# anisanazim/Movie-Recommendation-Engine

Measured on AMD Instinct MI355X. Metric: item embeddings/sec + top-K ANN queries/sec, ML-25M d=256, 1/2/4/8 GPU, higher is better.
Workload: dtype f64 cdf / f32 features / fp4 sign planes (exact integer Hamming); 1 GPU; SYN-25M (ML-25M-shaped: U=162541 M=59047 R=25000095), F=128 H=256 d=256, 2 GCN layers, W=100 L=2 T=10, LSH 512-bit, 10000 queries K=11, rng=numpy (the reference's np.random MT19937 stream generated on device: neighbour ids bit-exact with the reference CPU path); global_items=59047, queries=10000, parallelism=item-shard x1

## Files before the change

### include/pinsage_hip.h

```cpp
#ifndef PINSAGE_HIP_H
#define PINSAGE_HIP_H

#include <stddef.h>
#include <stdint.h>

#ifdef __cplusplus
extern "C" {
#endif

#define PS_OK 0
#define PS_EINVAL (-1)
#define PS_ELAUNCH (-2)
#define PS_EWORKSPACE (-3)
#define PS_EUNSUPPORTED (-4)

#define PS_RNG_STREAM 0
#define PS_RNG_PHILOX 1
#define PS_RNG_STREAM_RAW 2

#define PS_RNG_STREAM_WALKS 3

#define PS_WALK_HALF_BUCKETS 0x100

typedef void *ps_stream_t;

int ps_abi_version(void);
const char *ps_error_string(int code);

size_t ps_csr_build_workspace_bytes(int64_t E, int64_t V);
int ps_csr_build(const int64_t *src, const int64_t *dst, const float *w, int64_t E, int64_t V,
                 int64_t *rowptr, int32_t *col, double *wsorted,
                 void *workspace, size_t workspace_bytes, ps_stream_t stream);

int ps_cdf_build(const int64_t *rowptr, const double *wsorted, int64_t V, double *cdf, ps_stream_t stream);

int ps_guide_build(const int64_t *rowptr, const double *cdf, int64_t V, uint32_t *nodeinfo, int32_t *guide,
                   ps_stream_t stream);

int ps_pack_edges(const int32_t *col, const double *cdf, const int32_t *guide, int64_t E, void *packed,
                  ps_stream_t stream);

int ps_bucket_build(const int64_t *rowptr, const int32_t *col, const double *cdf, const int32_t *guide, int64_t V,
                    int64_t E, void *buckets, ps_stream_t stream);

int ps_bucket_build_half(const int64_t *rowptr, const int32_t *col, const double *cdf, const int32_t *guide, int64_t V,
                         int64_t E, void *buckets, ps_stream_t stream);

int ps_dest_info_build(const int32_t *col, const uint32_t *nodeinfo, int64_t E, int64_t V, void *dest_info, ps_stream_t stream);

int ps_graph_stats(const int64_t *rowptr, const int32_t *col, int64_t E, int64_t V, int64_t *flags,
                   ps_stream_t stream);

int ps_walk_sample(const int64_t *rowptr, const int32_t *col, const double *cdf, int64_t V,
                   const int64_t *starts, int64_t B, int W, int L, int T,
                   int rng_mode, const double *uniforms, const int64_t *uoff,
                   uint64_t seed, uint32_t call, const uint32_t *nodeinfo, const int32_t *guide,
                   const void *packed, const void *buckets, const void *dest_info,
                   int32_t *ids, int32_t *counts, int32_t *nvalid, ps_stream_t stream);

int ps_walk_sample_layers(const int64_t *rowptr, const int32_t *col, const double *cdf, int64_t V,
                          const int64_t *starts, int64_t B, int W, int L, int T,
                          int rng_mode, const double *uniforms, const int64_t *uoff, int64_t layer_stride,
                          uint64_t seed, uint32_t call, const uint32_t *nodeinfo, const int32_t *guide,
                          const void *packed, const void *buckets, const void *dest_info, int layers,
                          int32_t *ids, int32_t *counts, int32_t *nvalid, ps_stream_t stream);

int ps_walk_paths(const int64_t *rowptr, const int32_t *col, const double *cdf, int64_t V,
                  const int64_t *starts, int64_t B, int L, int rng_mode, const double *uniforms,
                  const int64_t *uoff, uint64_t seed, uint32_t call, int walk_mod,
                  const uint32_t *nodeinfo, const int32_t *guide, int32_t *paths, ps_stream_t stream);

int ps_uniform_offsets(const int64_t *rowptr, int64_t V, const int64_t *starts, int64_t B, int W, int L,
                       int64_t *uoff, int64_t *total, ps_stream_t stream);

int ps_mt19937_chunk_log2(void);
int ps_mt19937_window_shift(void);
int ps_mt19937_raw_stream(const uint32_t *state_in, int pos_in, int64_t n, uint32_t *raw, uint32_t *state_out,
                          int32_t *pos_out, const uint32_t *jump_polys, int jump_levels, const uint32_t *radix_polys,
                          int radix_levels, const uint32_t *window_polys, int n_window, const int64_t *ranges,
                          int n_ranges, void *workspace, size_t workspace_bytes, ps_stream_t stream);
size_t ps_mt19937_workspace_bytes(int64_t skip, int64_t n);
int ps_mt19937_random_sample(const uint32_t *state_in, int pos_in, int64_t skip, int64_t n, double *out,
                             uint32_t *state_out, int32_t *pos_out, const uint32_t *jump_polys, int jump_levels,
                             const uint32_t *radix_polys, int radix_levels, const uint32_t *window_polys, int n_window,
                             void *workspace, size_t workspace_bytes, ps_stream_t stream);

int ps_importance_pool(const float *x, int64_t N, int H, const int32_t *ids, const int32_t *counts,
                       const float *wts, const int32_t *nvalid, int64_t B, int T, int64_t max_idx,
                       int renorm, float *out, ps_stream_t stream);

#define PS_RELU 1
#define PS_L2NORM 2
#define PS_WPERM 4
int ps_permute_k(const float *W, int64_t rows, int K, int ld, float *out, ps_stream_t stream);
int ps_linear(const float *x, int64_t M, int K, const float *W, int ldw, const float *b, int N,
              const float *x2, int K2, const float *W2, int ldw2, int flags, float *y, ps_stream_t stream);

int ps_lsh_encode(const float *x, int64_t N, int D, const float *A, int nbits, uint8_t *codes, int flags, ps_stream_t stream);

size_t ps_hamming_topk_workspace_bytes(int64_t nq, int64_t N, int cs, int k);
int ps_hamming_topk(const uint8_t *qcodes, int64_t nq, const uint8_t *codes, int64_t N, int cs, int k,
                    int64_t id_offset, int32_t *dist, int64_t *ids,
                    void *workspace, size_t workspace_bytes, ps_stream_t stream);

size_t ps_lsh_planes_bytes(int64_t n, int cs);
int ps_lsh_expand(const uint8_t *codes, int64_t n, int cs, void *planes, ps_stream_t stream);
size_t ps_hamming_topk_mfma_workspace_bytes(int64_t nq, int64_t N, int cs, int k);
int ps_hamming_topk_mfma(const void *qplanes, int64_t nq, const void *dbplanes, int64_t N, int cs, int k,
                         int64_t id_offset, int32_t *dist, int64_t *ids,
                         void *workspace, size_t workspace_bytes, ps_stream_t stream);
int ps_hamming_topk_mfma_codes(const uint8_t *qcodes, int64_t nq, const void *dbplanes, int64_t N, int cs, int k,
                               int64_t id_offset, int32_t *dist, int64_t *ids,
                               void *workspace, size_t workspace_bytes, ps_stream_t stream);

int ps_topk_merge(const int32_t *dist_in, const int64_t *ids_in, int P, int64_t nq, int k,
                  int32_t *dist, int64_t *ids, ps_stream_t stream);
int ps_topk_merge_strided(const int32_t *dist_in, int64_t dist_stride, const int64_t *ids_in, int64_t ids_stride,
                          int P, int64_t nq, int k, int32_t *dist, int64_t *ids, ps_stream_t stream);

size_t ps_dot_topk_workspace_bytes(int64_t nq, int64_t N, int D, int k);
int ps_dot_topk(const float *E, int64_t N, int D, const int64_t *qidx, int64_t nq, int k, int exclude_self,
                float *vals, int64_t *ids, void *workspace, size_t workspace_bytes, ps_stream_t stream);

size_t ps_l2_topk_workspace_bytes(int64_t nq, int64_t N, int D, int k);
int ps_l2_topk(const float *X, int64_t N, int D, const float *Q, int64_t nq, int k, const int32_t *assign,
               const uint32_t *probe, int words, float *dist, int64_t *ids, void *workspace,
               size_t workspace_bytes, ps_stream_t stream);

size_t ps_ivf_topk_workspace_bytes(int64_t nq, int64_t N, int D, int k, int nlist, int nprobe, int64_t max_list);
int ps_ivf_topk(const float *X, int64_t N, int D, const int64_t *list_ptr, int nlist, int64_t max_list,
                const int64_t *item_ids, const float *Q, int64_t nq, const int32_t *probes, int nprobe, int k,
                float *dist, int64_t *ids, void *workspace, size_t workspace_bytes, ps_stream_t stream);

int ps_spmm_csr(const int64_t *rowptr, const int32_t *col, const float *val, const float *x, int64_t N, int H,
                int64_t V, int64_t E, float *out, ps_stream_t stream);

#ifdef __cplusplus
}
#endif
#endif
```

### movie-recommendation-engine_amd/csrc/dense_mfma.hip

```cpp
#include "ps_common.h"
#include <type_traits>

#ifndef PS_GEMM_DEBUG
#define PS_GEMM_DEBUG 0
#endif

#ifndef PS_GEMM_SPREAD
#define PS_GEMM_SPREAD 1
#endif

#if PS_GEMM_DEBUG & 64
__device__ unsigned long long ps_gemm_trace_buf[4096 * 4 * 48];
#define PS_TRACE(slot) do { if (lane == 0 && blockIdx.x < 4096 && (slot) < 48) \
    ps_gemm_trace_buf[((size_t)blockIdx.x * 4 + (wv & 3)) * 48 + (slot)] = __builtin_readcyclecounter(); } while (0)
extern "C" int ps_debug_gemm_trace(unsigned long long *host, int clear) {
    if (clear) { static unsigned long long z[4096 * 4 * 48]; return (int)hipMemcpyToSymbol(HIP_SYMBOL(ps_gemm_trace_buf), z, sizeof z); }
    return (int)hipMemcpyFromSymbol(host, HIP_SYMBOL(ps_gemm_trace_buf), sizeof(unsigned long long) * 4096 * 4 * 48);
}
#else
#define PS_TRACE(slot) do {} while (0)
#endif

namespace {

typedef float f32x16 __attribute__((ext_vector_type(16)));
typedef float f32x4 __attribute__((ext_vector_type(4)));


struct GemmArgs {
    const float *x;  int64_t M; int K;  const float *W;  int ldw;
    const float *x2; int K2;            const float *W2; int ldw2;
    const float *bias; int N; int flags;
    float *y;
    uint8_t *codes; int cs;
    const int64_t *grp;
};

__device__ __forceinline__ void load8(const float *base, bool row_ok, int k, int K, bool vec_ok, float (&v)[8]) {
    if (row_ok && vec_ok && k + 8 <= K) {
        const float4 a = *reinterpret_cast<const float4 *>(base + k);
        const float4 b = *reinterpret_cast<const float4 *>(base + k + 4);
        v[0] = a.x; v[1] = a.y; v[2] = a.z; v[3] = a.w; v[4] = b.x; v[5] = b.y; v[6] = b.z; v[7] = b.w;
    } else {
#pragma unroll
        for (int j = 0; j < 8; ++j) v[j] = (row_ok && k + j < K) ? base[k + j] : 0.f;
    }
}

#define PS_DPP_ACC(v, ctrl, rows) \
    (v) += __builtin_bit_cast(float, __builtin_amdgcn_update_dpp(0, __builtin_bit_cast(int, (v)), (ctrl), (rows), 0xf, true))
__device__ __forceinline__ float half_sum32(float v) {
    PS_DPP_ACC(v, 0xB1, 0xf);
    PS_DPP_ACC(v, 0x4E, 0xf);
    PS_DPP_ACC(v, 0x141, 0xf);
    PS_DPP_ACC(v, 0x140, 0xf);
    PS_DPP_ACC(v, 0x142, 0xa);
    return v;
}
#undef PS_DPP_ACC

#define PS_DPP_ADD(v, ctrl) \
    ((v) + __builtin_bit_cast(float, __builtin_amdgcn_update_dpp(0, __builtin_bit_cast(int, (v)), (ctrl), 0xf, 0xf, true)))
template <int NV>
__device__ __forceinline__ float transpose_sum32(float (&v)[NV], int lane) {
    static_assert(NV == 16 || NV == 32, "one or two 32-row tiles per wave");
    const bool p1 = ((lane ^ (lane >> 2)) & 1) != 0, p2 = (((lane >> 1) ^ (lane >> 2)) & 1) != 0;
    const bool p3 = (((lane >> 2) ^ (lane >> 3)) & 1) != 0, p4 = ((lane >> 3) & 1) != 0;
#pragma unroll
    for (int j = 0; j < NV / 2; ++j) {
        const float lo = PS_DPP_ADD(v[2 * j], 0xB1), hi = PS_DPP_ADD(v[2 * j + 1], 0xB1);
        v[j] = p1 ? hi : lo;
    }
#pragma unroll
    for (int j = 0; j < NV / 4; ++j) {
        const float lo = PS_DPP_ADD(v[2 * j], 0x4E), hi = PS_DPP_ADD(v[2 * j + 1], 0x4E);
        v[j] = p2 ? hi : lo;
    }
#pragma unroll
    for (int j = 0; j < NV / 8; ++j) {
        const float lo = PS_DPP_ADD(v[2 * j], 0x141), hi = PS_DPP_ADD(v[2 * j + 1], 0x141);
        v[j] = p3 ? hi : lo;
    }
#pragma unroll
    for (int j = 0; j < NV / 16; ++j) {
        const float lo = PS_DPP_ADD(v[2 * j], 0x140), hi = PS_DPP_ADD(v[2 * j + 1], 0x140);
        v[j] = p4 ? hi : lo;
    }
    const float x = v[0], y = NV == 32 ? v[1] : v[0];
    const auto sw = __builtin_amdgcn_permlane16_swap(__builtin_bit_cast(unsigned, x), __builtin_bit_cast(unsigned, y), false, false);
    const unsigned s0 = sw[0], s1 = sw[1];
    return __builtin_bit_cast(float, s0) + __builtin_bit_cast(float, s1);
}
#undef PS_DPP_ADD

template <bool PIN>
__device__ __forceinline__ void stash_item(float *d, f32x4 lo, f32x4 hi) {
    if (PIN) asm volatile("" : "+v"(lo), "+v"(hi));
    *reinterpret_cast<f32x4 *>(d) = f32x4{lo[0], lo[2], hi[0], hi[2]};
    *reinterpret_cast<f32x4 *>(d + 4) = f32x4{lo[1], lo[3], hi[1], hi[3]};
}
template <bool PIN>
__device__ __forceinline__ void stash_item_stored(float *d, f32x4 lo, f32x4 hi) {
    if (PIN) asm volatile("" : "+v"(lo), "+v"(hi));
    *reinterpret_cast<f32x4 *>(d) = lo;
    *reinterpret_cast<f32x4 *>(d + 4) = hi;
}

template <int WM, int WN, int TM, int TN, int EPI>
__device__ __forceinline__ void gemm_epilogue(const GemmArgs &g, f32x16 (&acc)[TM][TN], int64_t m0, int n0, float *sRed, float *sNrm) {
    constexpr int BM = WM * TM * 32, BN = WN * TN * 32, NT = WM * WN * 64;
    const int tid = threadIdx.x, lane = tid & 63, wv = tid >> 6;
    const int wm = wv / WN, wn = wv % WN, li = lane & 31, lh = lane >> 5;
    (void)BN; (void)wv;
    PS_TRACE(40);
    if (EPI == 1) {
        uint32_t *codes32 = reinterpret_cast<uint32_t *>(g.codes);
        const int words = g.cs >> 2;
#pragma unroll
        for (int a = 0; a < TM; ++a)
#pragma unroll
            for (int b = 0; b < TN; ++b) {
                const int colbase = n0 + (wn * TN + b) * 32;
                const bool col_ok = colbase + li < g.N;
#pragma unroll
                for (int r = 0; r < 16; ++r) {
                    const uint64_t mask = __ballot(col_ok && acc[a][b][r] >= 0.f);
                    const int64_t row = m0 + (wm * TM + a) * 32 + (r & 3) + 8 * (r >> 2) + 4 * lh;
                    if (li == 0 && row < g.M && colbase < g.N)
                        codes32[row * words + (colbase >> 5)] = lh ? (uint32_t)(mask >> 32) : (uint32_t)mask;
                }
            }
        PS_TRACE(41);
        return;
    }

    const bool relu = (g.flags & PS_RELU) && !(PS_GEMM_DEBUG & 8), l2 = (g.flags & PS_L2NORM) && !(PS_GEMM_DEBUG & 8);
    if (PS_GEMM_DEBUG & 32) {
        float s = 0.f;
#pragma unroll
        for (int a = 0; a < TM; ++a)
#pragma unroll
            for (int b = 0; b < TN; ++b)
#pragma unroll
                for (int r = 0; r < 16; ++r) s += acc[a][b][r];
        if (s == 12345.678f) g.y[0] = s;
        PS_TRACE(41);
        return;
    }
#pragma unroll
    for (int b = 0; b < TN; ++b) {
        const int col = n0 + (wn * TN + b) * 32 + li;
        const float bv = (g.bias && col < g.N) ? g.bias[col] : 0.f;
#pragma unroll
        for (int a = 0; a < TM; ++a)
#pragma unroll
            for (int r = 0; r < 16; ++r) {
                float v = acc[a][b][r] + bv;
                if (relu) v = v > 0.f ? v : 0.f;
                if (col >= g.N) v = 0.f;
                acc[a][b][r] = v;
            }
    }
    PS_TRACE(42);
    if (l2) {
        float ss[TM * 16];
#pragma unroll
        for (int a = 0; a < TM; ++a)
#pragma unroll
            for (int r = 0; r < 16; ++r) {
                float t = 0.f;
#pragma unroll
                for (int b = 0; b < TN; ++b) t = fmaf(acc[a][b][r], acc[a][b][r], t);
                ss[a * 16 + r] = t;
            }
        const float tot = transpose_sum32<TM * 16>(ss, lane);
        {
            const int idx = ((lane ^ (lane >> 2)) & 1) | (((lane >> 1) ^ (lane >> 2)) & 1) << 1 | (((lane >> 2) ^ (lane >> 3)) & 1) << 2 |
                            (lane & 8) | (TM == 2 ? lane & 16 : 0);
            const int a = idx >> 4, r = idx & 15;
            const int rowl = (wm * TM + a) * 32 + (r & 3) + 8 * (r >> 2) + 4 * lh;
            if (TM == 2 || li < 16) sRed[rowl * WN + wn] = tot;
        }
        PS_TRACE(43);
        __syncthreads();
        for (int row = tid; row < BM; row += NT) {
            float t = 0.f;
#pragma unroll
            for (int w = 0; w < WN; ++w) t += sRed[row * WN + w];
            float nrm = sqrtf(t);
            nrm = nrm > 1e-12f ? nrm : 1e-12f;
            const bool tame = nrm >= 0x1p-40f && nrm <= 0x1p40f;
            *reinterpret_cast<f32x4 *>(sNrm + row * 4) = f32x4{nrm, 1.0f / nrm, nrm * 0x1p-60f, tame ? 0.f : 1.f};
        }
        __syncthreads();
        PS_TRACE(44);
        bool wild = false;
#pragma unroll
        for (int a = 0; a < TM; ++a)
#pragma unroll
            for (int r = 0; r < 16; ++r) {
                const f32x4 nr = *reinterpret_cast<const f32x4 *>(sNrm + ((wm * TM + a) * 32 + (r & 3) + 8 * (r >> 2) + 4 * lh) * 4);
                wild |= nr[3] != 0.f;
#pragma unroll
                for (int b = 0; b < TN; ++b)
                    wild |= __float_as_uint(acc[a][b][r]) != 0u && !(fabsf(acc[a][b][r]) >= nr[2]);
            }
        if (__builtin_amdgcn_ballot_w64(wild) == 0) {
#pragma unroll
            for (int a = 0; a < TM; ++a)
#pragma unroll
                for (int r = 0; r < 16; ++r) {
                    const f32x4 nr = *reinterpret_cast<const f32x4 *>(sNrm + ((wm * TM + a) * 32 + (r & 3) + 8 * (r >> 2) + 4 * lh) * 4);
                    const float nrm = nr[0], y = nr[1];
#pragma unroll
                    for (int b = 0; b < TN; ++b) {
                        const float x = acc[a][b][r];
                        const float q0 = x * y, q1 = fmaf(fmaf(-nrm, q0, x), y, q0);
                        acc[a][b][r] = fmaf(fmaf(-nrm, q1, x), y, q1);
                    }
                }
        } else {
#pragma unroll
            for (int a = 0; a < TM; ++a)
#pragma unroll
                for (int r = 0; r < 16; ++r) {
                    const float nrm = sNrm[((wm * TM + a) * 32 + (r & 3) + 8 * (r >> 2) + 4 * lh) * 4];
#pragma unroll
                    for (int b = 0; b < TN; ++b) acc[a][b][r] = acc[a][b][r] / nrm;
                }
        }
    }
    PS_TRACE(45);
    const bool interior = (m0 + BM <= g.M) && (n0 + BN <= g.N);
    if (interior) {
#pragma unroll
        for (int a = 0; a < TM; ++a)
#pragma unroll
            for (int r = 0; r < 16; ++r) {
                float *dst = g.y + (m0 + (wm * TM + a) * 32 + (r & 3) + 8 * (r >> 2) + 4 * lh) * g.N + n0 + wn * TN * 32 + li;
#pragma unroll
                for (int b = 0; b < TN; ++b) dst[b * 32] = acc[a][b][r];
            }
        PS_TRACE(41);
        return;
    }
#pragma unroll
    for (int a = 0; a < TM; ++a)
#pragma unroll
        for (int r = 0; r < 16; ++r) {
            const int64_t row = m0 + (wm * TM + a) * 32 + (r & 3) + 8 * (r >> 2) + 4 * lh;
            if (row >= g.M) continue;
#pragma unroll
            for (int b = 0; b < TN; ++b) {
                const int col = n0 + (wn * TN + b) * 32 + li;
                if (col < g.N) g.y[row * g.N + col] = acc[a][b][r];
            }
        }
    PS_TRACE(41);
}

template <int WM, int WN, int TM, int TN, int BK, int EPI, bool FAST>
#ifndef PS_GEMM_OCC
#define PS_GEMM_OCC 2
#endif
__global__ __launch_bounds__(WM * WN * 64, PS_GEMM_OCC) void gemm_f32_kernel(GemmArgs g_in) {
    GemmArgs g = g_in;
    constexpr int BM = WM * TM * 32, BN = WN * TN * 32, NT = WM * WN * 64;
    constexpr bool SPREAD = FAST && PS_GEMM_SPREAD && TM * TN >= 4;
    constexpr int GRP = BK / 8;
    constexpr int LDS_STRIDE = BK + 4;
    constexpr int A_ITEMS = (BM * GRP + NT - 1) / NT, B_ITEMS = (BN * GRP + NT - 1) / NT;
    __shared__ __attribute__((aligned(16))) float smem[(BM + BN) * LDS_STRIDE + BM * WN + BM * 4];
    float *sA = smem, *sB = smem + BM * LDS_STRIDE, *sRed = smem + (BM + BN) * LDS_STRIDE, *sNrm = sRed + BM * WN;

    const int tid = threadIdx.x, lane = tid & 63, wv = tid >> 6;
    const int wm = wv / WN, wn = wv % WN;
    const int64_t m0 = (int64_t)blockIdx.x * BM;
    const int n0 = blockIdx.y * BN;
    const int li = lane & 31, lh = lane >> 5;
    if (g.grp != nullptr) {
        const int64_t *d = g.grp + (size_t)blockIdx.x * 3;
        const int64_t w_row0 = d[0], ncols = d[1], y_off = d[2];
        if (n0 >= ncols) return;
        g.W += w_row0 * g.ldw;
        g.N = (int)ncols;
        g.y += y_off - m0 * ncols;
    }

#if PS_GEMM_DEBUG & 64
    if (lane == 0 && blockIdx.x < 4096) {
        ps_gemm_trace_buf[((size_t)blockIdx.x * 4 + (wv & 3)) * 48 + 46] = __builtin_amdgcn_s_getreg((32 - 1) << 11 | 4);
        ps_gemm_trace_buf[((size_t)blockIdx.x * 4 + (wv & 3)) * 48 + 47] = __builtin_amdgcn_s_getreg((4 - 1) << 11 | 20);
    }
    int trace_step = 0;
#endif
    PS_TRACE(0);
    f32x16 acc[TM][TN];
#pragma unroll
    for (int a = 0; a < TM; ++a)
#pragma unroll
        for (int b = 0; b < TN; ++b)
#pragma unroll
            for (int r = 0; r < 16; ++r) acc[a][b][r] = 0.f;

    for (int phase = 0; phase < 2; ++phase) {
        const float *X = phase == 0 ? g.x : g.x2;
        const float *Wp = phase == 0 ? g.W : g.W2;
        const int K = phase == 0 ? g.K : g.K2;
        const int ldw = phase == 0 ? g.ldw : g.ldw2;
        if (X == nullptr || K <= 0) continue;
        const bool vecA = (K % 4 == 0) && (reinterpret_cast<size_t>(X) % 16 == 0);
        const bool vecB = (ldw % 4 == 0) && (reinterpret_cast<size_t>(Wp) % 16 == 0);

        const bool wperm = (g.flags & PS_WPERM) != 0;
        f32x4 ra[A_ITEMS][2], rb[B_ITEMS][2];
        auto fetch = [&](int k0) {
#pragma unroll
            for (int q = 0; q < A_ITEMS; ++q) {
                const int it = FAST ? (tid + NT * q) % (BM * GRP) : tid + NT * q, row = it / GRP, grp = it % GRP;
                const int64_t m = m0 + row;
                if (FAST) {
                    const float *src = X + (m < g.M ? m : g.M - 1) * K + k0 + grp * 8;
                    ra[q][0] = *reinterpret_cast<const f32x4 *>(src);
                    ra[q][1] = *reinterpret_cast<const f32x4 *>(src + 4);
                } else if (it < BM * GRP) {
                    float v[8];
                    load8(X + m * K, m < g.M, k0 + grp * 8, K, vecA, v);
#pragma unroll
                    for (int j = 0; j < 4; ++j) { ra[q][0][j] = v[j]; ra[q][1][j] = v[4 + j]; }
                }
            }
#pragma unroll
            for (int q = 0; q < B_ITEMS; ++q) {
                const int it = FAST ? (tid + NT * q) % (BN * GRP) : tid + NT * q, row = it / GRP, grp = it % GRP;
                const int n = n0 + row;
                if (FAST) {
                    const float *src = Wp + (int64_t)(n < g.N ? n : g.N - 1) * ldw + k0 + grp * 8;
                    rb[q][0] = *reinterpret_cast<const f32x4 *>(src);
                    rb[q][1] = *reinterpret_cast<const f32x4 *>(src + 4);
                } else if (it < BN * GRP) {
                    float v[8];
                    load8(Wp + (int64_t)n * ldw, n < g.N, k0 + grp * 8, K, vecB, v);
#pragma unroll
                    for (int j = 0; j < 4; ++j) { rb[q][0][j] = v[j]; rb[q][1][j] = v[4 + j]; }
                }
            }
        };
        auto stash = [&]() {
#pragma unroll
            for (int q = 0; q < A_ITEMS; ++q) {
                const int it = FAST ? (tid + NT * q) % (BM * GRP) : tid + NT * q, row = it / GRP, grp = it % GRP;
                if (!FAST && it >= BM * GRP) continue;
                float *d = sA + row * LDS_STRIDE + grp * 8;
                stash_item<SPREAD>(d, ra[q][0], ra[q][1]);
            }
#pragma unroll
            for (int q = 0; q < B_ITEMS; ++q) {
                const int it = FAST ? (tid + NT * q) % (BN * GRP) : tid + NT * q, row = it / GRP, grp = it % GRP;
                if (!FAST && it >= BN * GRP) continue;
                float *d = sB + row * LDS_STRIDE + grp * 8;
                if (FAST && wperm) stash_item_stored<SPREAD>(d, rb[q][0], rb[q][1]);
                else stash_item<SPREAD>(d, rb[q][0], rb[q][1]);
            }
        };

        fetch(0);
        for (int k0 = 0; k0 < K; k0 += BK) {
#if PS_GEMM_DEBUG & 64
            PS_TRACE(2 + 2 * trace_step);
#endif
            if (!(PS_GEMM_DEBUG & 4) || k0 == 0) __syncthreads();
            if (!(PS_GEMM_DEBUG & 2) || k0 == 0) stash();
            if (!(PS_GEMM_DEBUG & 4) || k0 == 0) __syncthreads();
#if PS_GEMM_DEBUG & 64
            PS_TRACE(3 + 2 * trace_step);
            ++trace_step;
#endif
            if (SPREAD && !(PS_GEMM_DEBUG & 1)) fetch(k0 + BK < K ? k0 + BK : k0);
            else if (k0 + BK < K && !(PS_GEMM_DEBUG & 1)) fetch(k0 + BK);
            f32x4 fa[2][TM], fb[2][TN];
            auto frags = [&](int grp, int s) {
#pragma unroll
                for (int a = 0; a < TM; ++a)
                    fa[s][a] = *reinterpret_cast<const f32x4 *>(sA + ((wm * TM + a) * 32 + li) * LDS_STRIDE + grp * 8 + lh * 4);
#pragma unroll
                for (int b = 0; b < TN; ++b)
                    fb[s][b] = *reinterpret_cast<const f32x4 *>(sB + ((wn * TN + b) * 32 + li) * LDS_STRIDE + grp * 8 + lh * 4);
            };
            if (!(PS_GEMM_DEBUG & 16) || k0 == 0) frags(0, 0);
#pragma unroll
            for (int grp = 0; grp < GRP; ++grp) {
                const int s = (PS_GEMM_DEBUG & 16) ? 0 : grp & 1;
                if (grp + 1 < GRP && !(PS_GEMM_DEBUG & 16)) frags(grp + 1, s ^ 1);
#pragma unroll
                for (int t = 0; t < 4; ++t)
#pragma unroll
                    for (int a = 0; a < TM; ++a)
#pragma unroll
                        for (int b = 0; b < TN; ++b)
                            acc[a][b] = __builtin_amdgcn_mfma_f32_32x32x2f32(fa[s][a][t], fb[s][b][t], acc[a][b], 0, 0, 0);
            }
            __builtin_amdgcn_sched_group_barrier(0x100, TM + TN, 0);
#pragma unroll
            for (int grp = 0; grp < GRP; ++grp) {
                if (grp + 1 < GRP) __builtin_amdgcn_sched_group_barrier(0x100, TM + TN, 0);
#pragma unroll
                for (int t = 0; t < 4; ++t) {
                    __builtin_amdgcn_sched_group_barrier(0x008, TM * TN, 0);
                    if (SPREAD) __builtin_amdgcn_sched_group_barrier(0x020, 1, 0);
                }
            }
        }
    }

    gemm_epilogue<WM, WN, TM, TN, EPI>(g, acc, m0, n0, sRed, sNrm);
}

template <int WM, int WN, int TM, int TN, int BK, int EPI>
__global__ __launch_bounds__(WM * WN * 64, PS_GEMM_OCC) void gemm_f32_pkernel(GemmArgs g, int tiles_n, int ntiles) {
    constexpr int BM = WM * TM * 32, BN = WN * TN * 32, NT = WM * WN * 64;
    constexpr bool SPREAD = PS_GEMM_SPREAD && TM * TN >= 4;
    constexpr int GRP = BK / 8;
    constexpr int LDS_STRIDE = BK + 4;
    constexpr int A_ITEMS = (BM * GRP + NT - 1) / NT, B_ITEMS = (BN * GRP + NT - 1) / NT;
    __shared__ __attribute__((aligned(16))) float smem[(BM + BN) * LDS_STRIDE + BM * WN + BM * 4];
    float *sA = smem, *sB = smem + BM * LDS_STRIDE, *sRed = smem + (BM + BN) * LDS_STRIDE, *sNrm = sRed + BM * WN;
    const int tid = threadIdx.x, lane = tid & 63, wv = tid >> 6;
    const int wm = wv / WN, wn = wv % WN;
    const int li = lane & 31, lh = lane >> 5;
    const int steps0 = g.K / BK, steps1 = g.x2 != nullptr ? g.K2 / BK : 0, nsteps = steps0 + steps1;
    const bool wperm = (g.flags & PS_WPERM) != 0;

    f32x4 ra[A_ITEMS][2], rb[B_ITEMS][2];
    auto fetch = [&](int64_t m0, int n0, int s) __attribute__((always_inline)) {
        const bool second = s >= steps0;
        const float *X = second ? g.x2 : g.x;
        const float *Wp = second ? g.W2 : g.W;
        const int K = second ? g.K2 : g.K, ldw = second ? g.ldw2 : g.ldw;
        const int k0 = (second ? s - steps0 : s) * BK;
#pragma unroll
        for (int q = 0; q < A_ITEMS; ++q) {
            const int it = (tid + NT * q) % (BM * GRP), row = it / GRP, grp = it % GRP;
            const int64_t m = m0 + row;
            const float *src = X + (m < g.M ? m : g.M - 1) * K + k0 + grp * 8;
            ra[q][0] = *reinterpret_cast<const f32x4 *>(src);
            ra[q][1] = *reinterpret_cast<const f32x4 *>(src + 4);
        }
#pragma unroll
        for (int q = 0; q < B_ITEMS; ++q) {
            const int it = (tid + NT * q) % (BN * GRP), row = it / GRP, grp = it % GRP;
            const int n = n0 + row;
            const float *src = Wp + (int64_t)(n < g.N ? n : g.N - 1) * ldw + k0 + grp * 8;
            rb[q][0] = *reinterpret_cast<const f32x4 *>(src);
            rb[q][1] = *reinterpret_cast<const f32x4 *>(src + 4);
        }
    };
    auto stash = [&]() __attribute__((always_inline)) {
#pragma unroll
        for (int q = 0; q < A_ITEMS; ++q) {
            const int it = (tid + NT * q) % (BM * GRP), row = it / GRP, grp = it % GRP;
            stash_item<SPREAD>(sA + row * LDS_STRIDE + grp * 8, ra[q][0], ra[q][1]);
        }
#pragma unroll
        for (int q = 0; q < B_ITEMS; ++q) {
            const int it = (tid + NT * q) % (BN * GRP), row = it / GRP, grp = it % GRP;
            if (wperm) stash_item_stored<SPREAD>(sB + row * LDS_STRIDE + grp * 8, rb[q][0], rb[q][1]);
            else stash_item<SPREAD>(sB + row * LDS_STRIDE + grp * 8, rb[q][0], rb[q][1]);
        }
    };

    int tile = blockIdx.x;
    if (tile >= ntiles) return;
    int64_t m0 = (int64_t)(tile / tiles_n) * BM;
    int n0 = (tile % tiles_n) * BN;
    fetch(m0, n0, 0);
    while (true) {
        const int next = tile + (int)gridDim.x;
        const bool more = next < ntiles;
        const int64_t m0n = more ? (int64_t)(next / tiles_n) * BM : m0;
        const int n0n = more ? (next % tiles_n) * BN : n0;
        f32x16 acc[TM][TN];
#pragma unroll
        for (int a = 0; a < TM; ++a)
#pragma unroll
            for (int b = 0; b < TN; ++b)
#pragma unroll
                for (int r = 0; r < 16; ++r) acc[a][b][r] = 0.f;
        for (int s = 0; s < nsteps; ++s) {
            __syncthreads();
            stash();
            __syncthreads();
            {
                const bool last = s + 1 >= nsteps;
                fetch(last ? m0n : m0, last ? n0n : n0, last ? (more ? 0 : s) : s + 1);
            }
            f32x4 fa[2][TM], fb[2][TN];
            auto frags = [&](int grp, int sl) __attribute__((always_inline)) {
#pragma unroll
                for (int a = 0; a < TM; ++a)
                    fa[sl][a] = *reinterpret_cast<const f32x4 *>(sA + ((wm * TM + a) * 32 + li) * LDS_STRIDE + grp * 8 + lh * 4);
#pragma unroll
                for (int b = 0; b < TN; ++b)
                    fb[sl][b] = *reinterpret_cast<const f32x4 *>(sB + ((wn * TN + b) * 32 + li) * LDS_STRIDE + grp * 8 + lh * 4);
            };
            frags(0, 0);
#pragma unroll
            for (int grp = 0; grp < GRP; ++grp) {
                const int sl = grp & 1;
                if (grp + 1 < GRP) frags(grp + 1, sl ^ 1);
#pragma unroll
                for (int t = 0; t < 4; ++t)
#pragma unroll
                    for (int a = 0; a < TM; ++a)
#pragma unroll
                        for (int b = 0; b < TN; ++b)
                            acc[a][b] = __builtin_amdgcn_mfma_f32_32x32x2f32(fa[sl][a][t], fb[sl][b][t], acc[a][b], 0, 0, 0);
            }
            __builtin_amdgcn_sched_group_barrier(0x100, TM + TN, 0);
#pragma unroll
            for (int grp = 0; grp < GRP; ++grp) {
                if (grp + 1 < GRP) __builtin_amdgcn_sched_group_barrier(0x100, TM + TN, 0);
#pragma unroll
                for (int t = 0; t < 4; ++t) {
                    __builtin_amdgcn_sched_group_barrier(0x008, TM * TN, 0);
                    if (SPREAD) __builtin_amdgcn_sched_group_barrier(0x020, 1, 0);
                }
            }
        }
        gemm_epilogue<WM, WN, TM, TN, EPI>(g, acc, m0, n0, sRed, sNrm);
        if (!more) break;
        tile = next;
        m0 = m0n;
        n0 = n0n;
    }
}

#pragma clang diagnostic push
#pragma clang diagnostic ignored "-Winline-asm"
__device__ __forceinline__ void gemm_lds_dma16(const void *gptr, uint32_t lds_byte_offset) {
    asm volatile("s_mov_b32 m0, %1\n\tglobal_load_lds_dwordx4 %0, off" ::"v"(gptr), "s"(lds_byte_offset) : "memory", "m0");
}
#pragma clang diagnostic pop

constexpr int DMA_BM = 64, DMA_BN = 256, DMA_BK = 32, DMA_STAGES = 2, DMA_WAVES = 4;
constexpr int DMA_STAGE_BYTES = (DMA_BM + DMA_BN) * DMA_BK * 4;
constexpr int DMA_APIECES = DMA_BM / 64 * (DMA_BK / 4);
constexpr int DMA_PIECES = (DMA_BM + DMA_BN) / 64 * (DMA_BK / 4);
constexpr int DMA_PPW = DMA_PIECES / DMA_WAVES;

template <int EPI>
__global__ __launch_bounds__(DMA_WAVES * 64, 2) void gemm_dma_kernel(GemmArgs g) {
    extern __shared__ __attribute__((aligned(1024))) unsigned char dsm[];
    const int tid = threadIdx.x, lane = tid & 63;
    const int wv = __builtin_amdgcn_readfirstlane(tid >> 6);
    const int wm = 0, wn = wv;
    const int li = lane & 31, lh = lane >> 5;
    const int64_t m0 = (int64_t)blockIdx.x * DMA_BM;
    const int n0 = blockIdx.y * DMA_BN;
    const uint32_t lds_base = (uint32_t)reinterpret_cast<uintptr_t>(dsm);
    const int nk1 = g.K / DMA_BK, nk2 = (g.x2 ? g.K2 : 0) / DMA_BK, nks = nk1 + nk2;

    f32x16 acc[2][2];
#pragma unroll
    for (int a = 0; a < 2; ++a)
#pragma unroll
        for (int b = 0; b < 2; ++b)
#pragma unroll
            for (int r = 0; r < 16; ++r) acc[a][b][r] = 0.f;

    const unsigned char *src[DMA_PPW];
    auto sources = [&](bool second) {
        const float *X = second ? g.x2 : g.x;
        const float *Wp = second ? g.W2 : g.W;
        const int K = second ? g.K2 : g.K;
        const int ldw = second ? g.ldw2 : g.ldw;
#pragma unroll
        for (int q = 0; q < DMA_PPW; ++q) {
            const int p = wv + DMA_WAVES * q;
            const int kk = p & 7;
            if (p < DMA_APIECES) {
                int64_t row = m0 + lane;
                row = row < g.M ? row : g.M - 1;
                src[q] = reinterpret_cast<const unsigned char *>(X + row * K + kk * 4);
            } else {
                int n = n0 + ((p - DMA_APIECES) >> 3) * 64 + lane;
                n = n < g.N ? n : g.N - 1;
                src[q] = reinterpret_cast<const unsigned char *>(Wp + (int64_t)n * ldw + kk * 4);
            }
        }
    };
    auto prefetch = [&](int ks, int buf) {
        const int kbytes = (ks >= nk1 ? ks - nk1 : ks) * (DMA_BK * 4);
#pragma unroll
        for (int q = 0; q < DMA_PPW; ++q)
            gemm_lds_dma16(src[q] + kbytes, lds_base + (uint32_t)(buf * DMA_STAGE_BYTES + (wv + DMA_WAVES * q) * 1024));
    };

    sources(nk1 == 0);
    __builtin_amdgcn_s_waitcnt(0x0F70);
    if (nks > 0) prefetch(0, 0);
    int buf = 0;
    for (int ks = 0; ks < nks; ++ks) {
        asm volatile("s_waitcnt vmcnt(0)" ::: "memory");
        __builtin_amdgcn_s_barrier();
        if (ks + 1 < nks) {
            if (ks + 1 == nk1) sources(true);
            prefetch(ks + 1, buf ^ 1);
        }
        const unsigned char *sA = dsm + buf * DMA_STAGE_BYTES + (wm * 8) * 1024 + li * 16;
        const unsigned char *sB = dsm + buf * DMA_STAGE_BYTES + (DMA_APIECES + wn * 8) * 1024 + li * 16;
        float4 fa[2][2], fb[2][2];
        auto frags = [&](int kk, int s) {
#pragma unroll
            for (int a = 0; a < 2; ++a) fa[s][a] = *reinterpret_cast<const float4 *>(sA + kk * 1024 + a * 512);
#pragma unroll
            for (int b = 0; b < 2; ++b) fb[s][b] = *reinterpret_cast<const float4 *>(sB + kk * 1024 + b * 512);
        };
        frags(0, 0);
        __builtin_amdgcn_sched_group_barrier(0x100, 4, 0);
#pragma unroll
        for (int kk = 0; kk < DMA_BK / 4; ++kk) {
            const int s = kk & 1;
            if (kk + 1 < DMA_BK / 4) {
                frags(kk + 1, s ^ 1);
                __builtin_amdgcn_sched_group_barrier(0x100, 4, 0);
            }
#pragma unroll
            for (int m = 0; m < 2; ++m) {
                float av[2], bv[2];
#pragma unroll
                for (int a = 0; a < 2; ++a) av[a] = m == 0 ? (lh ? fa[s][a].y : fa[s][a].x) : (lh ? fa[s][a].w : fa[s][a].z);
#pragma unroll
                for (int b = 0; b < 2; ++b) bv[b] = m == 0 ? (lh ? fb[s][b].y : fb[s][b].x) : (lh ? fb[s][b].w : fb[s][b].z);
#pragma unroll
                for (int a = 0; a < 2; ++a)
#pragma unroll
                    for (int b = 0; b < 2; ++b) acc[a][b] = __builtin_amdgcn_mfma_f32_32x32x2f32(av[a], bv[b], acc[a][b], 0, 0, 0);
            }
        }
        buf ^= 1;
    }

    if (EPI == 1) {
        uint32_t *codes32 = reinterpret_cast<uint32_t *>(g.codes);
        const int words = g.cs >> 2;
#pragma unroll
        for (int a = 0; a < 2; ++a)
#pragma unroll
            for (int b = 0; b < 2; ++b) {
                const int colbase = n0 + (wn * 2 + b) * 32;
                const bool col_ok = colbase + li < g.N;
#pragma unroll
                for (int r = 0; r < 16; ++r) {
                    const uint64_t mask = __ballot(col_ok && acc[a][b][r] >= 0.f);
                    const int64_t row = m0 + (wm * 2 + a) * 32 + (r & 3) + 8 * (r >> 2) + 4 * lh;
                    if (li == 0 && row < g.M && colbase < g.N)
                        codes32[row * words + (colbase >> 5)] = lh ? (uint32_t)(mask >> 32) : (uint32_t)mask;
                }
            }
        return;
    }
    const bool relu = g.flags & PS_RELU, l2 = g.flags & PS_L2NORM;
#pragma unroll
    for (int b = 0; b < 2; ++b) {
        const int col = n0 + (wn * 2 + b) * 32 + li;
        const float bias = (g.bias && col < g.N) ? g.bias[col] : 0.f;
#pragma unroll
        for (int a = 0; a < 2; ++a)
#pragma unroll
            for (int r = 0; r < 16; ++r) {
                float v = acc[a][b][r] + bias;
                if (relu) v = v > 0.f ? v : 0.f;
                if (col >= g.N) v = 0.f;
                acc[a][b][r] = v;
            }
    }
    if (l2) {
        float *sRed = reinterpret_cast<float *>(dsm);
        __syncthreads();
#pragma unroll
        for (int a = 0; a < 2; ++a)
#pragma unroll
            for (int r = 0; r < 16; ++r) {
                float ss = 0.f;
#pragma unroll
                for (int b = 0; b < 2; ++b) ss = fmaf(acc[a][b][r], acc[a][b][r], ss);
                ss = half_sum32(ss);
                const int rowl = (wm * 2 + a) * 32 + (r & 3) + 8 * (r >> 2) + 4 * lh;
                if (li == 16) sRed[rowl * 4 + wn] = ss;
            }
        __syncthreads();
#pragma unroll
        for (int a = 0; a < 2; ++a)
#pragma unroll
            for (int r = 0; r < 16; ++r) {
                const int rowl = (wm * 2 + a) * 32 + (r & 3) + 8 * (r >> 2) + 4 * lh;
                float ss = 0.f;
#pragma unroll
                for (int w = 0; w < 4; ++w) ss += sRed[rowl * 4 + w];
                float nrm = sqrtf(ss);
                nrm = nrm > 1e-12f ? nrm : 1e-12f;
#pragma unroll
                for (int b = 0; b < 2; ++b) acc[a][b][r] = acc[a][b][r] / nrm;
            }
    }
#pragma unroll
    for (int a = 0; a < 2; ++a)
#pragma unroll
        for (int r = 0; r < 16; ++r) {
            const int64_t row = m0 + (wm * 2 + a) * 32 + (r & 3) + 8 * (r >> 2) + 4 * lh;
            if (row >= g.M) continue;
#pragma unroll
            for (int b = 0; b < 2; ++b) {
                const int col = n0 + (wn * 2 + b) * 32 + li;
                if (col < g.N) g.y[row * g.N + col] = acc[a][b][r];
            }
        }
}

constexpr int SH_BM = 32, SH_BN = 256, SH_BK = 32;
constexpr int SH_STAGE_BYTES = (SH_BM + SH_BN) * SH_BK * 4;
constexpr int SH_TAIL_BYTES = (SH_BM * 4 + SH_BM * 4) * 4;

#pragma clang diagnostic push
#pragma clang diagnostic ignored "-Winline-asm"
__device__ __forceinline__ void shard_lds_dma16(uint32_t voff, const void *sbase, uint32_t lds_byte_offset) {
    asm volatile("s_mov_b32 m0, %2\n\tglobal_load_lds_dwordx4 %0, %1" ::"v"(voff), "s"(sbase), "s"(lds_byte_offset) : "memory", "m0");
}
#pragma clang diagnostic pop

template <int EPI, bool WP, int STAGES>
__global__ __launch_bounds__(256, STAGES == 2 ? 2 : 1) void gemm_shard_kernel(GemmArgs g) {
    static_assert(STAGES == 2 || STAGES == 3, "ring of two or three images");
    extern __shared__ __attribute__((aligned(1024))) unsigned char dsm[];
    const int tid = threadIdx.x, lane = tid & 63;
    const int wv = __builtin_amdgcn_readfirstlane(tid >> 6);
    const int wn = wv;
    const int li = lane & 31, lh = lane >> 5;
    const int64_t m0 = (int64_t)blockIdx.x * SH_BM;
    const int n0 = blockIdx.y * SH_BN;
    const uint32_t lds_base = (uint32_t)reinterpret_cast<uintptr_t>(dsm);
    const int nk1 = g.K / SH_BK, nk2 = (g.x2 ? g.K2 : 0) / SH_BK, nks = nk1 + nk2;
    float *sRed = reinterpret_cast<float *>(dsm + STAGES * SH_STAGE_BYTES), *sNrm = sRed + SH_BM * 4;

    f32x16 acc[1][2];
#pragma unroll
    for (int b = 0; b < 2; ++b)
#pragma unroll
        for (int r = 0; r < 16; ++r) acc[0][b][r] = 0.f;

    uint32_t voff[9];
    auto offsets = [&](bool second) {
        const int K = second ? g.K2 : g.K, ldw = second ? g.ldw2 : g.ldw;
        int64_t row = m0 + li;
        row = (row < g.M ? row : g.M - 1) - m0;
        voff[0] = (uint32_t)row * (uint32_t)K * 4u + (uint32_t)(2 * wv + lh) * 16u;
#pragma unroll
        for (int q = 1; q < 9; ++q) {
            const int idx = wv + 4 * (q - 1);
            int n = n0 + (idx >> 3) * 64 + lane;
            n = (n < g.N ? n : g.N - 1) - n0;
            voff[q] = (uint32_t)n * (uint32_t)ldw * 4u + (uint32_t)(idx & 7) * 16u;
        }
    };
    const float *Xc = g.x + m0 * g.K, *Wc = g.W + (int64_t)n0 * g.ldw;
    const float *X2c = g.x2 ? g.x2 + m0 * g.K2 : nullptr, *W2c = g.x2 ? g.W2 + (int64_t)n0 * g.ldw2 : nullptr;
    uint32_t issue_lds = 0;
    auto issue_begin = [&](int ks, int buf) {
        if (ks == nk1) {
            offsets(true);
            Xc = X2c;
            Wc = W2c;
        }
        issue_lds = lds_base + (uint32_t)(buf * SH_STAGE_BYTES + wv * 1024);
    };
    auto issue_piece = [&](int q) {
        shard_lds_dma16(voff[q], q == 0 ? Xc : Wc, issue_lds + (uint32_t)q * 4096u);
        if (q == 8) {
            Xc += SH_BK;
            Wc += SH_BK;
        }
    };
    auto issue = [&](int ks, int buf) {
        issue_begin(ks, buf);
#pragma unroll
        for (int q = 0; q < 9; ++q) issue_piece(q);
    };

#if PS_GEMM_DEBUG & 64
    const unsigned long long tr_start = __builtin_readcyclecounter();
    unsigned long long tr_wait = 0, tr_first = 0, tr_stream = 0, tr_a = 0, tr_b = 0, tr_c = 0;
#endif
    offsets(false);
    __builtin_amdgcn_s_waitcnt(0x0F70);
    issue(0, 0);
    if (STAGES == 3 && nks > 1) issue(1, 1);
    int buf = 0;
    for (int ks = 0; ks < nks; ++ks) {
#if PS_GEMM_DEBUG & 64
        tr_a = __builtin_readcyclecounter();
        if (ks > 0) tr_stream += tr_a - tr_c;
#endif
        if (STAGES == 3 && ks + 1 < nks) asm volatile("s_waitcnt vmcnt(9)" ::: "memory");
        else asm volatile("s_waitcnt vmcnt(0)" ::: "memory");
        __builtin_amdgcn_s_barrier();
#if PS_GEMM_DEBUG & 64
        tr_b = __builtin_readcyclecounter();
        tr_wait += tr_b - tr_a;
#endif
        const unsigned char *sA = dsm + buf * SH_STAGE_BYTES + li * 16 + lh * 4;
        const unsigned char *sB = dsm + buf * SH_STAGE_BYTES + (4 + wn * 8) * 1024 + li * 16 + (WP ? lh * 1024 : lh * 4);
        float av[2][4];
        f32x4 bv[2][2];
        auto frags = [&](int grp, int s) {
#pragma unroll
            for (int h = 0; h < 2; ++h) {
                const float *p = reinterpret_cast<const float *>(sA + grp * 1024 + h * 512);
                av[s][2 * h] = p[0];
                av[s][2 * h + 1] = p[2];
            }
#pragma unroll
            for (int b = 0; b < 2; ++b) {
                if (WP) {
                    bv[s][b] = *reinterpret_cast<const f32x4 *>(sB + 2 * grp * 1024 + b * 512);
                } else {
#pragma unroll
                    for (int h = 0; h < 2; ++h) {
                        const float *p = reinterpret_cast<const float *>(sB + (2 * grp + h) * 1024 + b * 512);
                        bv[s][b][2 * h] = p[0];
                        bv[s][b][2 * h + 1] = p[2];
                    }
                }
            }
        };
        const int nx = ks + STAGES - 1;
        frags(0, 0);
        auto stream = [&](auto more_tag) __attribute__((always_inline)) {
            constexpr bool MORE = decltype(more_tag)::value;
            if (MORE) issue_begin(nx, buf == 0 ? STAGES - 1 : buf - 1);
            __builtin_amdgcn_sched_barrier(0);
#if PS_GEMM_DEBUG & 64
            asm volatile("s_waitcnt lgkmcnt(0)" ::: "memory");
            tr_c = __builtin_readcyclecounter();
            tr_first += tr_c - tr_b;
#endif
#pragma unroll
            for (int grp = 0; grp < SH_BK / 8; ++grp) {
                const int s = grp & 1;
                if (grp + 1 < SH_BK / 8) {
                    frags(grp + 1, s ^ 1);
                    __builtin_amdgcn_sched_barrier(0);
                }
#pragma unroll
                for (int t = 0; t < 4; ++t)
#pragma unroll
                    for (int b = 0; b < 2; ++b) {
                        acc[0][b] = __builtin_amdgcn_mfma_f32_32x32x2f32(av[s][t], bv[s][b][t], acc[0][b], 0, 0, 0);
                        const int q = grp * 8 + t * 2 + b;
                        if (MORE && q < 9) {
                            __builtin_amdgcn_sched_barrier(0);
                            issue_piece(q);
                            __builtin_amdgcn_sched_barrier(0);
                        }
                    }
            }
        };
        if (nx < nks) stream(std::true_type{});
        else stream(std::false_type{});
        buf = buf + 1 == STAGES ? 0 : buf + 1;
    }
#if PS_GEMM_DEBUG & 64
    if (lane == 0 && blockIdx.x < 4096 && blockIdx.y == 0) {
        unsigned long long *t = ps_gemm_trace_buf + ((size_t)blockIdx.x * 4 + wv) * 48;
        t[0] = tr_start; t[1] = tr_wait; t[2] = tr_first; t[3] = tr_stream + (__builtin_readcyclecounter() - tr_c);
        t[46] = __builtin_amdgcn_s_getreg((32 - 1) << 11 | 4); t[47] = __builtin_amdgcn_s_getreg((4 - 1) << 11 | 20);
    }
#endif
    gemm_epilogue<1, 4, 1, 2, EPI>(g, acc, m0, n0, sRed, sNrm);
}

__global__ void l2norm_rows_kernel(float *y, int64_t M, int N) {
    const int lane = threadIdx.x & 63;
    const int64_t wave = ((int64_t)blockIdx.x * blockDim.x + threadIdx.x) >> 6;
    const int64_t nw = ((int64_t)gridDim.x * blockDim.x) >> 6;
    for (int64_t m = wave; m < M; m += nw) {
        float ss = 0.f;
        for (int n = lane; n < N; n += 64) ss = fmaf(y[m * N + n], y[m * N + n], ss);
        ss = ps_wave_sum_f32(ss);
        float nrm = sqrtf(ss);
        nrm = nrm > 1e-12f ? nrm : 1e-12f;
        for (int n = lane; n < N; n += 64) y[m * N + n] = y[m * N + n] / nrm;
    }
}

template <typename K>
int persistent_slots(K kernel, PsPerDevice &slots) {
    int dv = 0;
    if (hipGetDevice(&dv) != hipSuccess || dv < 0 || dv >= 64) return 0;
    int n = slots.get(dv);
    if (n == 0) {
        int per_cu = 0, cus = 0;
        if (hipOccupancyMaxActiveBlocksPerMultiprocessor(&per_cu, kernel, 256, 0) != hipSuccess || per_cu <= 0) return 0;
        if (hipDeviceGetAttribute(&cus, hipDeviceAttributeMultiprocessorCount, dv) != hipSuccess || cus <= 0) return 0;
        n = per_cu * cus;
        slots.set(dv, n);
    }
    return n;
}

template <int WM, int WN, int TM, int TN, int EPI>
int launch_persistent(const GemmArgs &g, hipStream_t st) {
    constexpr int BM = WM * TM * 32, BN = WN * TN * 32;
    const int64_t tiles_m = ps_cdiv(g.M, BM);
    const int tiles_n = (int)ps_cdiv(g.N, BN);
    const int64_t ntiles = tiles_m * tiles_n;
    if (ntiles > 0x7fffffff) return PS_EUNSUPPORTED;
    static PsPerDevice slot_cache;
    const int slots = persistent_slots(gemm_f32_pkernel<WM, WN, TM, TN, 32, EPI>, slot_cache);
    if (slots <= 0) return PS_ELAUNCH;
    const unsigned grid = (unsigned)(ntiles < slots ? ntiles : slots);
    hipLaunchKernelGGL((gemm_f32_pkernel<WM, WN, TM, TN, 32, EPI>), dim3(grid), dim3(256), 0, st, g, tiles_n, (int)ntiles);
    PS_CHECK_LAUNCH();
    return PS_OK;
}

template <int EPI, bool FAST>
int launch_gemm_v(const GemmArgs &g, hipStream_t st) {
    if (FAST && g.grp == nullptr && g.N > 128 && (g.x2 == nullptr || g.K2 % 32 == 0)) {
        const char *pe = getenv("PS_GEMM_PERSIST");
        const bool persist = pe == nullptr || atoi(pe) != 0;
        if (persist) {
            if (!(g.flags & PS_L2NORM)) return launch_persistent<2, 2, 1, 2, EPI>(g, st);
            if (g.M < 64 * 384) return launch_persistent<1, 4, 1, 2, EPI>(g, st);
        }
    }
    if (g.N <= 64) {
        dim3 grid((unsigned)ps_cdiv(g.M, 64), 1);
        hipLaunchKernelGGL((gemm_f32_kernel<2, 2, 1, 1, 32, EPI, FAST>), grid, dim3(256), 0, st, g);
    } else if (g.N <= 128) {
        dim3 grid((unsigned)ps_cdiv(g.M, 64), 1);
        hipLaunchKernelGGL((gemm_f32_kernel<2, 2, 1, 2, 32, EPI, FAST>), grid, dim3(256), 0, st, g);
    } else {
        if (!(g.flags & PS_L2NORM)) {
            dim3 grid((unsigned)ps_cdiv(g.M, 64), (unsigned)ps_cdiv(g.N, 128));
            hipLaunchKernelGGL((gemm_f32_kernel<2, 2, 1, 2, 32, EPI, FAST>), grid, dim3(256), 0, st, g);
        } else if (g.M < 64 * 384) {
            dim3 grid((unsigned)ps_cdiv(g.M, 32), (unsigned)ps_cdiv(g.N, 256));
            hipLaunchKernelGGL((gemm_f32_kernel<1, 4, 1, 2, 32, EPI, FAST>), grid, dim3(256), 0, st, g);
        } else {
            dim3 grid((unsigned)ps_cdiv(g.M, 64), (unsigned)ps_cdiv(g.N, 256));
            hipLaunchKernelGGL((gemm_f32_kernel<1, 4, 2, 2, 32, EPI, FAST>), grid, dim3(256), 0, st, g);
        }
    }
    PS_CHECK_LAUNCH();
    return PS_OK;
}

bool aligned_operand(const float *p, int K, int ld) {
    return p == nullptr || (reinterpret_cast<size_t>(p) % 16 == 0 && K % 32 == 0 && ld % 4 == 0);
}

template <int EPI, bool WP, int STAGES>
int launch_shard(const GemmArgs &g, hipStream_t st) {
    constexpr int lds = STAGES * SH_STAGE_BYTES + SH_TAIL_BYTES;
    static PsPerDevice attr_done;
    int devid = 0;
    if (hipGetDevice(&devid) != hipSuccess || devid < 0 || devid >= 64) return PS_ELAUNCH;
    if (!attr_done.get(devid)) {
        if (hipFuncSetAttribute(reinterpret_cast<const void *>(gemm_shard_kernel<EPI, WP, STAGES>),
                                hipFuncAttributeMaxDynamicSharedMemorySize, lds) != hipSuccess) return PS_ELAUNCH;
        attr_done.set(devid, 1);
    }
    dim3 grid((unsigned)ps_cdiv(g.M, SH_BM), (unsigned)ps_cdiv(g.N, SH_BN));
    hipLaunchKernelGGL((gemm_shard_kernel<EPI, WP, STAGES>), grid, dim3(256), lds, st, g);
    PS_CHECK_LAUNCH();
    return PS_OK;
}

constexpr int64_t SHARD_TILES_RING3 = 256, SHARD_TILES_RING2 = 512;

template <int EPI>
int launch_gemm(const GemmArgs &g, hipStream_t st) {
    const bool fast = aligned_operand(g.x, g.K, g.K) && aligned_operand(g.W, g.K, g.ldw) &&
                      (g.x2 == nullptr || (aligned_operand(g.x2, g.K2, g.K2) && aligned_operand(g.W2, g.K2, g.ldw2)));
    {
        const char *se = getenv("PS_GEMM_SHARD");
        const int mode = se ? atoi(se) : -1;
        const int64_t tiles = ps_cdiv(g.M, SH_BM) * ps_cdiv(g.N, SH_BN);
        const bool fits = (int64_t)g.ldw * 1024 < 0x7fffffff && (g.x2 == nullptr || (int64_t)g.ldw2 * 1024 < 0x7fffffff) &&
                          (int64_t)g.K * 128 < 0x7fffffff && (g.x2 == nullptr || (int64_t)g.K2 * 128 < 0x7fffffff);
        const bool by_size = EPI == 0 && (g.flags & PS_L2NORM) && tiles <= SHARD_TILES_RING2;
        if (fast && fits && g.grp == nullptr && g.N > 128 && mode != 0 && (mode > 0 || by_size)) {
            const bool wp = (g.flags & PS_WPERM) != 0;
            if (mode == 3 || (mode < 0 && tiles <= SHARD_TILES_RING3))
                return wp ? launch_shard<EPI, true, 3>(g, st) : launch_shard<EPI, false, 3>(g, st);
            return wp ? launch_shard<EPI, true, 2>(g, st) : launch_shard<EPI, false, 2>(g, st);
        }
    }
    const bool use_dma = getenv("PS_GEMM_DMA") != nullptr;
    if (fast && use_dma && !(g.flags & PS_WPERM) && g.N % DMA_BN == 0 && g.M >= 64 * 384) {
        static PsPerDevice attr_done;
        int devid = 0;
        if (hipGetDevice(&devid) != hipSuccess || devid < 0 || devid >= 64) return PS_ELAUNCH;
        if (!attr_done.get(devid)) {
            if (hipFuncSetAttribute(reinterpret_cast<const void *>(gemm_dma_kernel<EPI>), hipFuncAttributeMaxDynamicSharedMemorySize,
                                    DMA_STAGES * DMA_STAGE_BYTES) != hipSuccess) return PS_ELAUNCH;
            attr_done.set(devid, 1);
        }
        dim3 grid((unsigned)ps_cdiv(g.M, DMA_BM), (unsigned)(g.N / DMA_BN));
        hipLaunchKernelGGL((gemm_dma_kernel<EPI>), grid, dim3(DMA_WAVES * 64), DMA_STAGES * DMA_STAGE_BYTES, st, g);
        PS_CHECK_LAUNCH();
        return PS_OK;
    }
    if ((g.flags & PS_WPERM) && !fast) return PS_EINVAL;
    return fast ? launch_gemm_v<EPI, true>(g, st) : launch_gemm_v<EPI, false>(g, st);
}

}

int psi_linear_grouped(const float *x, int64_t M, int K, const float *W, int ldw, float *y, const int64_t *grp, int max_cols,
                       ps_stream_t stream) {
    if (M <= 0 || M % 64 != 0 || K <= 0 || max_cols <= 0 || !x || !W || !y || !grp || ldw < K) return PS_EINVAL;
    GemmArgs g{x, M, K, W, ldw, nullptr, 0, nullptr, 0, nullptr, max_cols, 0, y, nullptr, 0, grp};
    hipStream_t st = ps_stream(stream);
    dim3 grid((unsigned)(M / 64), (unsigned)ps_cdiv(max_cols, 128));
    if (aligned_operand(x, K, K) && aligned_operand(W, K, ldw))
        hipLaunchKernelGGL((gemm_f32_kernel<2, 2, 1, 2, 32, 0, true>), grid, dim3(256), 0, st, g);
    else
        hipLaunchKernelGGL((gemm_f32_kernel<2, 2, 1, 2, 32, 0, false>), grid, dim3(256), 0, st, g);
    PS_CHECK_LAUNCH();
    return PS_OK;
}

extern "C" int ps_linear(const float *x, int64_t M, int K, const float *W, int ldw, const float *b, int N,
                         const float *x2, int K2, const float *W2, int ldw2, int flags, float *y, ps_stream_t stream) {
    if (M < 0 || K <= 0 || N <= 0 || ldw < K) return PS_EINVAL;
    if (M == 0) return PS_OK;
    if (!x || !W || !y) return PS_EINVAL;
    if (x2 && (!W2 || K2 <= 0 || ldw2 < K2)) return PS_EINVAL;
    if (M > (int64_t)0x7fffffff * 64) return PS_EINVAL;
    hipStream_t st = ps_stream(stream);
    GemmArgs g{x, M, K, W, ldw, x2, x2 ? K2 : 0, W2, ldw2, b, N, flags, y, nullptr, 0};
    const bool fused_norm = N <= 256;
    if (!fused_norm) g.flags &= ~PS_L2NORM;
    int rc = launch_gemm<0>(g, st);
    if (rc != PS_OK) return rc;
    if ((flags & PS_L2NORM) && !fused_norm) {
        int64_t grid = ps_cdiv(M, 4);
        if (grid > 4096) grid = 4096;
        hipLaunchKernelGGL(l2norm_rows_kernel, dim3((unsigned)grid), dim3(256), 0, st, y, M, N);
        PS_CHECK_LAUNCH();
    }
    return PS_OK;
}

__global__ void permute_k_kernel(const float *__restrict__ W, int64_t rows, int K, int ld, float *__restrict__ out) {
    const int64_t total = rows * (K / 8);
    for (int64_t i = (int64_t)blockIdx.x * blockDim.x + threadIdx.x; i < total; i += (int64_t)gridDim.x * blockDim.x) {
        const int64_t r = i / (K / 8);
        const int g8 = (int)(i % (K / 8));
        const float *src = W + r * ld + g8 * 8;
        float *dst = out + r * K + g8 * 8;
#pragma unroll
        for (int j = 0; j < 4; ++j) { dst[j] = src[2 * j]; dst[4 + j] = src[2 * j + 1]; }
    }
}

extern "C" int ps_permute_k(const float *W, int64_t rows, int K, int ld, float *out, ps_stream_t stream) {
    if (rows < 0 || K <= 0 || K % 8 != 0 || ld < K) return PS_EINVAL;
    if (rows == 0) return PS_OK;
    if (!W || !out) return PS_EINVAL;
    int64_t grid = ps_cdiv(rows * (K / 8), 256);
    if (grid > 4096) grid = 4096;
    hipLaunchKernelGGL(permute_k_kernel, dim3((unsigned)grid), dim3(256), 0, ps_stream(stream), W, rows, K, ld, out);
    PS_CHECK_LAUNCH();
    return PS_OK;
}

extern "C" int ps_lsh_encode(const float *x, int64_t N, int D, const float *A, int nbits, uint8_t *codes, int flags,
                             ps_stream_t stream) {
    if (N < 0 || D <= 0 || nbits <= 0 || (flags & ~PS_WPERM)) return PS_EINVAL;
    if (nbits % 32 != 0) return PS_EUNSUPPORTED;
    if (N == 0) return PS_OK;
    if (!x || !A || !codes || reinterpret_cast<size_t>(codes) % 4 != 0) return PS_EINVAL;
    GemmArgs g{x, N, D, A, D, nullptr, 0, nullptr, 0, nullptr, nbits, flags, nullptr, codes, nbits / 8};
    return launch_gemm<1>(g, ps_stream(stream));
}
```

### movie-recommendation-engine_amd/csrc/importance_pool.hip

```cpp
#include "ps_common.h"

namespace {

constexpr int UNROLL = 8;

template <int VEC>
__global__ __launch_bounds__(256) void importance_pool_kernel(const float *__restrict__ x, int H,
                                                              const int32_t *__restrict__ ids,
                                                              const int32_t *__restrict__ counts,
                                                              const float *__restrict__ wts,
                                                              const int32_t *__restrict__ nvalid, int64_t B, int T,
                                                              int64_t max_idx, int renorm,
                                                              float *__restrict__ out) {
    const int lane = threadIdx.x & 63;
    const int wave = __builtin_amdgcn_readfirstlane((int)((blockIdx.x * blockDim.x + threadIdx.x) >> 6));
    const int nwaves = (int)((gridDim.x * blockDim.x) >> 6);
    const int chunk = 64 * VEC;
    for (int64_t i = wave; i < B; i += nwaves) {
        const bool small = T <= 64;
        int32_t id0 = -1, cnt0 = 0;
        float wt0 = 0.f;
        if (small && lane < T) {
            id0 = ids[i * T + lane];
            if (counts) cnt0 = counts[i * T + lane];
            if (wts) wt0 = wts[i * T + lane];
        }
        const int k = __builtin_amdgcn_readfirstlane(nvalid[i]);
        int tot = 0;
        if (small) {
            tot = lane < k ? cnt0 : 0;
        } else {
            for (int j0 = 0; j0 < k; j0 += 64) {
                const int j = j0 + lane;
                tot += (counts && j < k) ? counts[i * T + j] : 0;
            }
        }
        tot = ps_wave_sum_i32(tot);
        float wsum = 0.f;
        if (small) {
            if (lane < k && id0 >= 0 && (int64_t)id0 <= max_idx) wsum = wts ? wt0 : (float)((double)cnt0 / (double)tot);
        } else {
            for (int j0 = 0; j0 < k; j0 += 64) {
                const int j = j0 + lane;
                float wj = 0.f;
                if (j < k) {
                    const int32_t id = ids[i * T + j];
                    if (id >= 0 && (int64_t)id <= max_idx)
                        wj = wts ? wts[i * T + j] : (float)((double)counts[i * T + j] / (double)tot);
                }
                wsum += wj;
            }
        }
        wsum = ps_wave_sum_f32(wsum);
        const bool do_norm = renorm && wsum > 0.f;
        for (int c0 = 0; c0 < H; c0 += chunk) {
            const int col = c0 + lane * VEC;
            const bool cact = col < H;
            float acc[VEC];
#pragma unroll
            for (int v = 0; v < VEC; ++v) acc[v] = 0.f;
            for (int j0 = 0; j0 < k; j0 += 64) {
                const int jj = j0 + lane;
                int32_t myid = -1;
                float myw = 0.f;
                if (jj < k) {
                    myid = small ? id0 : ids[i * T + jj];
                    if (myid >= 0 && (int64_t)myid <= max_idx) {
                        if (small) myw = wts ? wt0 : (float)((double)cnt0 / (double)tot);
                        else myw = wts ? wts[i * T + jj] : (float)((double)counts[i * T + jj] / (double)tot);
                        if (do_norm) myw = myw / wsum;
                    } else {
                        myid = -1;
                    }
                }
                const int kk = (k - j0) < 64 ? (k - j0) : 64;
                for (int t0 = 0; t0 < kk; t0 += UNROLL) {
                    float r[UNROLL][VEC];
                    float wv[UNROLL];
#pragma unroll
                    for (int u = 0; u < UNROLL; ++u) {
                        const int t = t0 + u;
                        const int32_t id = (t < kk) ? __builtin_amdgcn_readlane(myid, t < 64 ? t : 0) : -1;
                        wv[u] = (t < kk) ? __builtin_bit_cast(float, __builtin_amdgcn_readlane(__builtin_bit_cast(int, myw), t < 64 ? t : 0)) : 0.f;
                        const bool ok = id >= 0 && cact;
                        if (VEC == 4) {
                            float4 q = make_float4(0.f, 0.f, 0.f, 0.f);
                            if (ok) q = *reinterpret_cast<const float4 *>(x + (int64_t)id * H + col);
                            r[u][0] = q.x; r[u][1 % VEC] = q.y; r[u][2 % VEC] = q.z; r[u][3 % VEC] = q.w;
                        } else {
                            r[u][0] = ok ? x[(int64_t)id * H + col] : 0.f;
                        }
                    }
#pragma unroll
                    for (int u = 0; u < UNROLL; ++u)
#pragma unroll
                        for (int v = 0; v < VEC; ++v) acc[v] = fmaf(r[u][v], wv[u], acc[v]);
                }
            }
            if (cact) {
                if (VEC == 4) {
                    *reinterpret_cast<float4 *>(out + i * H + col) = make_float4(acc[0], acc[1 % VEC], acc[2 % VEC], acc[3 % VEC]);
                } else {
                    out[i * H + col] = acc[0];
                }
            }
        }
    }
}

template <int CTRL>
__device__ __forceinline__ int row_bcast_i32(int v) { return __builtin_amdgcn_update_dpp(0, v, CTRL, 0xf, 0xf, false); }
__device__ __forceinline__ int row16_sum_i32(int v) {
    v += __builtin_amdgcn_update_dpp(0, v, 0xB1, 0xf, 0xf, true);
    v += __builtin_amdgcn_update_dpp(0, v, 0x4E, 0xf, 0xf, true);
    v += __builtin_amdgcn_update_dpp(0, v, 0x141, 0xf, 0xf, true);
    v += __builtin_amdgcn_update_dpp(0, v, 0x140, 0xf, 0xf, true);
    return v;
}
__device__ __forceinline__ float row16_sum_f32(float v) {
    v += __builtin_bit_cast(float, __builtin_amdgcn_update_dpp(0, __builtin_bit_cast(int, v), 0xB1, 0xf, 0xf, true));
    v += __builtin_bit_cast(float, __builtin_amdgcn_update_dpp(0, __builtin_bit_cast(int, v), 0x4E, 0xf, 0xf, true));
    v += __builtin_bit_cast(float, __builtin_amdgcn_update_dpp(0, __builtin_bit_cast(int, v), 0x141, 0xf, 0xf, true));
    v += __builtin_bit_cast(float, __builtin_amdgcn_update_dpp(0, __builtin_bit_cast(int, v), 0x140, 0xf, 0xf, true));
    return v;
}

template <int PAGES>
__global__ __launch_bounds__(256) void importance_pool4_kernel(const float *__restrict__ x, int H, const int32_t *__restrict__ ids,
                                                               const int32_t *__restrict__ counts, const float *__restrict__ wts,
                                                               const int32_t *__restrict__ nvalid, int64_t B, int T, int64_t max_idx,
                                                               int renorm, float *__restrict__ out) {
    constexpr int TU = 4;
    const int lane = threadIdx.x & 63, l = lane & 15, g = lane >> 4;
    const int64_t wave0 = ((int64_t)blockIdx.x * blockDim.x + threadIdx.x) >> 6;
    const int64_t nwaves = ((int64_t)gridDim.x * blockDim.x) >> 6;
    for (int64_t i0 = wave0 * 4; i0 < B; i0 += nwaves * 4) {
        const int64_t i = i0 + g;
        const bool rok = i < B;
        int k = rok ? nvalid[i] : 0;
        int32_t id[PAGES], cn[PAGES];
        float w[PAGES];
#pragma unroll
        for (int p = 0; p < PAGES; ++p) {
            const int e = p * 16 + l;
            const bool in = rok && e < T;
            id[p] = in ? ids[i * T + e] : -1;
            cn[p] = (in && counts) ? counts[i * T + e] : 0;
            w[p] = (in && wts) ? wts[i * T + e] : 0.f;
        }
        k = k < T ? k : T;
        int tot = 0;
#pragma unroll
        for (int p = 0; p < PAGES; ++p) tot += (p * 16 + l < k) ? cn[p] : 0;
        tot = row16_sum_i32(tot);
        float wsum = 0.f;
#pragma unroll
        for (int p = 0; p < PAGES; ++p) {
            const bool keep = (p * 16 + l < k) && id[p] >= 0 && (int64_t)id[p] <= max_idx;
            w[p] = keep ? (wts ? w[p] : (float)((double)cn[p] / (double)tot)) : 0.f;
            id[p] = keep ? id[p] : -1;
            wsum += w[p];
        }
        wsum = row16_sum_f32(wsum);
        if (renorm && wsum > 0.f) {
#pragma unroll
            for (int p = 0; p < PAGES; ++p) w[p] = id[p] >= 0 ? w[p] / wsum : 0.f;
        }
        int kmax = __builtin_amdgcn_readlane(k, 0);
        { const int k1 = __builtin_amdgcn_readlane(k, 16), k2 = __builtin_amdgcn_readlane(k, 32), k3 = __builtin_amdgcn_readlane(k, 48);
          kmax = kmax > k1 ? kmax : k1; kmax = kmax > k2 ? kmax : k2; kmax = kmax > k3 ? kmax : k3; }
        for (int cb = 0; cb < H; cb += 256) {
            float4 acc[4];
#pragma unroll
            for (int s = 0; s < 4; ++s) acc[s] = make_float4(0.f, 0.f, 0.f, 0.f);
#define PS_POOL_ENTRY(P, TT, U)                                                                            \
            {                                                                                              \
                nid[U] = row_bcast_i32<0x150 + (TT)>(id[P]);                                               \
                nw[U] = __builtin_bit_cast(float, row_bcast_i32<0x150 + (TT)>(__builtin_bit_cast(int, w[P]))); \
                _Pragma("unroll") for (int s = 0; s < 4; ++s) {                                            \
                    const int col = cb + s * 64 + l * 4;                                                   \
                    r[U][s] = make_float4(0.f, 0.f, 0.f, 0.f);                                             \
                    if (nid[U] >= 0 && col < H) r[U][s] = *reinterpret_cast<const float4 *>(x + (int64_t)nid[U] * H + col); \
                }                                                                                          \
            }
#define PS_POOL_BATCH(P, T0)                                                                               \
            if ((P) * 16 + (T0) < kmax) {                                                                  \
                int32_t nid[TU];                                                                           \
                float nw[TU];                                                                              \
                float4 r[TU][4];                                                                           \
                PS_POOL_ENTRY(P, (T0) + 0, 0) PS_POOL_ENTRY(P, (T0) + 1, 1) PS_POOL_ENTRY(P, (T0) + 2, 2) PS_POOL_ENTRY(P, (T0) + 3, 3) \
                _Pragma("unroll") for (int u = 0; u < TU; ++u)                                             \
                    _Pragma("unroll") for (int s = 0; s < 4; ++s) {                                        \
                        acc[s].x = fmaf(r[u][s].x, nw[u], acc[s].x); acc[s].y = fmaf(r[u][s].y, nw[u], acc[s].y); \
                        acc[s].z = fmaf(r[u][s].z, nw[u], acc[s].z); acc[s].w = fmaf(r[u][s].w, nw[u], acc[s].w); \
                    }                                                                                      \
            }
#define PS_POOL_PAGE(P) PS_POOL_BATCH(P, 0) PS_POOL_BATCH(P, 4) PS_POOL_BATCH(P, 8) PS_POOL_BATCH(P, 12)
            PS_POOL_PAGE(0)
            if constexpr (PAGES > 1) { PS_POOL_PAGE(1) }
            if constexpr (PAGES > 2) { PS_POOL_PAGE(2) }
            if constexpr (PAGES > 3) { PS_POOL_PAGE(3) }
#undef PS_POOL_PAGE
#undef PS_POOL_BATCH
#undef PS_POOL_ENTRY
            if (rok) {
#pragma unroll
                for (int s = 0; s < 4; ++s) {
                    const int col = cb + s * 64 + l * 4;
                    if (col < H) *reinterpret_cast<float4 *>(out + i * H + col) = acc[s];
                }
            }
        }
    }
}

}

extern "C" int ps_importance_pool(const float *x, int64_t N, int H, const int32_t *ids, const int32_t *counts,
                                  const float *wts, const int32_t *nvalid, int64_t B, int T, int64_t max_idx,
                                  int renorm, float *out, ps_stream_t stream) {
    if (B < 0 || H <= 0 || T <= 0 || N < 0) return PS_EINVAL;
    if (B == 0) return PS_OK;
    if (!x || !ids || !nvalid || !out || (!counts && !wts)) return PS_EINVAL;
    if (max_idx > N - 1) max_idx = N - 1;
    int64_t grid = ps_cdiv(B, 4);
    if (grid > 256 * 16) grid = 256 * 16;
    hipStream_t st = ps_stream(stream);
    const bool vec4 = (H % 4 == 0) && ((reinterpret_cast<size_t>(x) | reinterpret_cast<size_t>(out)) % 16 == 0);
    const char *pe = getenv("PS_POOL_ROWS_PER_WAVE");
    const bool four = vec4 && T <= 64 && !(pe && atoi(pe) == 1);
    if (four) {
        int64_t g4 = ps_cdiv(B, 16);
        if (g4 > 256 * 64) g4 = 256 * 64;
        if (T <= 16)
            hipLaunchKernelGGL(importance_pool4_kernel<1>, dim3((unsigned)g4), dim3(256), 0, st, x, H, ids, counts, wts, nvalid, B, T,
                               max_idx, renorm, out);
        else
            hipLaunchKernelGGL(importance_pool4_kernel<4>, dim3((unsigned)g4), dim3(256), 0, st, x, H, ids, counts, wts, nvalid, B, T,
                               max_idx, renorm, out);
    } else if (vec4)
        hipLaunchKernelGGL(importance_pool_kernel<4>, dim3((unsigned)grid), dim3(256), 0, st, x, H, ids, counts, wts,
                           nvalid, B, T, max_idx, renorm, out);
    else
        hipLaunchKernelGGL(importance_pool_kernel<1>, dim3((unsigned)grid), dim3(256), 0, st, x, H, ids, counts, wts,
                           nvalid, B, T, max_idx, renorm, out);
    PS_CHECK_LAUNCH();
    return PS_OK;
}
```

### movie-recommendation-engine_amd/pinsage_hip/dense.py

```python
from __future__ import annotations

import os

import torch

from . import native as nv


def _rowmajor(w):
    if w.dtype != torch.float32:
        raise TypeError("fp32 expected")
    if w.dim() != 2:
        raise ValueError("2-D matrix expected")
    if w.stride(1) != 1 or w.stride(0) < w.size(1):
        w = w.contiguous()
    return w, int(w.stride(0)) if w.size(0) > 1 else max(int(w.stride(0)), int(w.size(1)))


def _require_cuda(*tensors):
    for t in tensors:
        if t is not None and not t.is_cuda:
            raise nv.NativeError("libpinsage_hip takes device (HBM) tensors; got a CPU tensor (no CPU fallback)")


def _ptr_view(t):
    if t is None:
        return nv.C.c_void_p(0)
    if not t.is_cuda:
        raise nv.NativeError("device tensor expected")
    return nv.C.c_void_p(t.data_ptr())


class StagedWeight:
    __slots__ = ("t", "shape")

    def __init__(self, t):
        self.t = t
        self.shape = t.shape

    def size(self, i):
        return self.t.size(i)


def stage_weight(W):
    if isinstance(W, StagedWeight) or W is None:
        return W
    _require_cuda(W)
    if W.dim() != 2 or W.dtype != torch.float32 or int(W.size(1)) % 32 != 0:
        return W
    Wk, ld = _rowmajor(W)
    out = torch.empty((int(Wk.size(0)), int(Wk.size(1))), dtype=torch.float32, device=W.device)
    with torch.cuda.device(W.device):
        nv.call("ps_permute_k", _ptr_view(Wk), nv.i64(int(Wk.size(0))), nv.i32(int(Wk.size(1))), nv.i32(ld), nv.ptr(out), nv.stream())
    return StagedWeight(out)


def linear(x, W, b=None, x2=None, W2=None, relu=False, l2norm=False):
    staged = isinstance(W, StagedWeight)
    if x2 is not None and isinstance(W2, StagedWeight) != staged:
        raise ValueError("W and W2 must both be staged or both plain")
    if staged:
        W, W2 = W.t, (W2.t if W2 is not None else None)
    _require_cuda(x, W, b, x2, W2)
    x = x.contiguous()
    if x.dtype != torch.float32:
        raise TypeError("fp32 expected")
    M, K = int(x.size(0)), int(x.size(1))
    Wk, ldw = _rowmajor(W)
    N = int(Wk.size(0))
    if int(Wk.size(1)) != K:
        raise ValueError(f"shape mismatch: x [{M},{K}] vs W {tuple(Wk.shape)}")
    K2, ldw2, W2k = 0, 0, None
    if x2 is not None:
        x2 = x2.contiguous()
        W2k, ldw2 = _rowmajor(W2)
        K2 = int(x2.size(1))
        if int(W2k.size(1)) != K2 or int(W2k.size(0)) != N or int(x2.size(0)) != M:
            raise ValueError("shape mismatch in the second operand pair")
    if b is not None:
        b = b.contiguous()
    y = torch.empty((M, N), dtype=torch.float32, device=x.device)
    flags = (nv.PS_RELU if relu else 0) | (nv.PS_L2NORM if l2norm else 0) | (nv.PS_WPERM if staged else 0)
    with torch.cuda.device(x.device):
        nv.call("ps_linear", nv.ptr(x), nv.i64(M), nv.i32(K), _ptr_view(Wk), nv.i32(ldw), nv.ptr(b), nv.i32(N),
                                    nv.ptr(x2), nv.i32(K2), _ptr_view(W2k), nv.i32(ldw2), nv.i32(flags), nv.ptr(y),
                                    nv.stream())
    return y


def lsh_encode(x, A):
    staged = isinstance(A, StagedWeight)
    if staged:
        A = A.t
    _require_cuda(x, A)
    x = x.contiguous()
    A = A.contiguous()
    n, d = int(x.size(0)), int(x.size(1))
    nbits = int(A.size(0))
    if int(A.size(1)) != d:
        raise ValueError("projection matrix must be [nbits, dim]")
    codes = torch.empty((n, nbits // 8), dtype=torch.uint8, device=x.device)
    with torch.cuda.device(x.device):
        nv.call("ps_lsh_encode", nv.ptr(x), nv.i64(n), nv.i32(d), nv.ptr(A), nv.i32(nbits), nv.ptr(codes),
                                        nv.i32(nv.PS_WPERM if staged else 0), nv.stream())
    return codes


HAMMING_MAX_K = 64


def lsh_expand(codes):
    _require_cuda(codes)
    codes = codes.contiguous()
    n, cs = int(codes.size(0)), int(codes.size(1))
    nb = int(nv.lib().ps_lsh_planes_bytes(nv.i64(n), nv.i32(cs)))
    if nb == 0:
        return None
    planes = torch.empty(nb, dtype=torch.uint8, device=codes.device)
    with torch.cuda.device(codes.device):
        nv.call("ps_lsh_expand", nv.ptr(codes), nv.i64(n), nv.i32(cs), nv.ptr(planes), nv.stream())
    return planes


def hamming_mfma_supported(nq, N, cs, k):
    return int(nv.lib().ps_hamming_topk_mfma_workspace_bytes(nv.i64(nq), nv.i64(N), nv.i32(cs), nv.i32(k))) > 0


def hamming_topk(qcodes, codes, k, id_offset=0, planes=None, use_mfma=True, out=None):
    _require_cuda(qcodes, codes)
    qcodes = qcodes.contiguous()
    codes = codes.contiguous()
    nq, cs = int(qcodes.size(0)), int(qcodes.size(1))
    N = int(codes.size(0))
    if out is not None:
        dist, ids = out
        if (tuple(dist.shape) != (nq, k) or tuple(ids.shape) != (nq, k) or dist.dtype != torch.int32
                or ids.dtype != torch.int64 or not dist.is_contiguous() or not ids.is_contiguous()):
            raise ValueError("out must be contiguous (int32 [nq, k], int64 [nq, k])")
    if k > HAMMING_MAX_K or cs > 128 or (cs & (cs - 1)) != 0 or cs % 4 != 0:
        d, i = _hamming_topk_large_k(qcodes, codes, k, id_offset)
        if out is None:
            return d, i
        dist.copy_(d)
        ids.copy_(i)
        return dist, ids
    if out is None:
        dist = torch.empty((nq, k), dtype=torch.int32, device=qcodes.device)
        ids = torch.empty((nq, k), dtype=torch.int64, device=qcodes.device)
    L = nv.lib()
    if use_mfma and planes is not None:
        wsb = int(L.ps_hamming_topk_mfma_workspace_bytes(nv.i64(nq), nv.i64(N), nv.i32(cs), nv.i32(k)))
        if wsb > 0:
            ws = torch.empty(wsb, dtype=torch.uint8, device=qcodes.device)
            with torch.cuda.device(qcodes.device):
                nv.call("ps_hamming_topk_mfma_codes", nv.ptr(qcodes), nv.i64(nq), nv.ptr(planes), nv.i64(N), nv.i32(cs),
                        nv.i32(k), nv.i64(id_offset), nv.ptr(dist), nv.ptr(ids), nv.ptr(ws), nv.C.c_size_t(wsb),
                        nv.stream())
            return dist, ids
    wsb = int(L.ps_hamming_topk_workspace_bytes(nv.i64(nq), nv.i64(N), nv.i32(cs), nv.i32(k)))
    ws = torch.empty(wsb, dtype=torch.uint8, device=qcodes.device)
    with torch.cuda.device(qcodes.device):
        nv.call("ps_hamming_topk", nv.ptr(qcodes), nv.i64(nq), nv.ptr(codes) if N else nv.C.c_void_p(0), nv.i64(N),
                                   nv.i32(cs), nv.i32(k), nv.i64(id_offset), nv.ptr(dist), nv.ptr(ids), nv.ptr(ws),
                                   nv.C.c_size_t(wsb), nv.stream())
    return dist, ids


LARGE_K_SIGN_BYTES = 8 << 30


def _signs(codes):
    shifts = torch.arange(8, device=codes.device, dtype=torch.uint8)
    bits = (codes.unsqueeze(-1) >> shifts) & 1
    return bits.reshape(codes.size(0), -1).to(torch.float32) * 2.0 - 1.0


def _hamming_topk_large_k(qcodes, codes, k, id_offset):
    N, nbits = int(codes.size(0)), int(codes.size(1)) * 8
    if N * nbits * 4 > LARGE_K_SIGN_BYTES:
        raise ValueError(f"LSH search with k = {k} > {HAMMING_MAX_K} expands the code table to floats "
                         f"({N * nbits * 4 / 2 ** 30:.1f} GiB here, limit {LARGE_K_SIGN_BYTES >> 30} GiB): split the table or the request")
    d2, ids = l2_topk(_signs(codes), _signs(qcodes), k)
    missing = ids < 0
    dist = torch.where(missing, torch.full_like(d2, 0.0), d2 * 0.25).round().to(torch.int32)
    dist[missing] = 0x7fffffff
    ids = torch.where(missing, ids, ids + int(id_offset))
    return dist, ids


def topk_merge(dist_in, ids_in):
    dist_in = dist_in.contiguous()
    ids_in = ids_in.contiguous()
    P, nq, k = [int(v) for v in dist_in.shape]
    dist = torch.empty((nq, k), dtype=torch.int32, device=dist_in.device)
    ids = torch.empty((nq, k), dtype=torch.int64, device=dist_in.device)
    with torch.cuda.device(dist_in.device):
        nv.call("ps_topk_merge", nv.ptr(dist_in), nv.ptr(ids_in), nv.i32(P), nv.i64(nq), nv.i32(k), nv.ptr(dist),
                                        nv.ptr(ids), nv.stream())
    return dist, ids


def topk_merge_records(records, nq, k):
    if records.dtype != torch.uint8 or records.dim() != 2 or not records.is_contiguous():
        raise ValueError("records must be a contiguous uint8 [P, record_bytes] tensor")
    P, rec = int(records.size(0)), int(records.size(1))
    n = int(nq) * int(k)
    if rec < 12 * n or rec % 8 != 0:
        raise ValueError("record too short or not 8-byte aligned")
    dist = torch.empty((nq, k), dtype=torch.int32, device=records.device)
    ids = torch.empty((nq, k), dtype=torch.int64, device=records.device)
    base = records.data_ptr()
    with torch.cuda.device(records.device):
        nv.call("ps_topk_merge_strided", nv.C.c_void_p(base + 8 * n), nv.i64(rec // 4), nv.C.c_void_p(base), nv.i64(rec // 8),
                nv.i32(P), nv.i64(int(nq)), nv.i32(int(k)), nv.ptr(dist), nv.ptr(ids), nv.stream())
    return dist, ids


def dot_topk(E, qidx, k, exclude_self=True):
    E = E.contiguous()
    qidx = qidx.to(device=E.device, dtype=torch.int64).contiguous()
    N, D = int(E.size(0)), int(E.size(1))
    nq = int(qidx.numel())
    if k < 1:
        raise ValueError(f"k must be positive, got {k}")
    vals = torch.empty((nq, k), dtype=torch.float32, device=E.device)
    ids = torch.empty((nq, k), dtype=torch.int64, device=E.device)
    L = nv.lib()
    wsb = int(L.ps_dot_topk_workspace_bytes(nv.i64(nq), nv.i64(N), nv.i32(D), nv.i32(k)))
    ws = torch.empty(wsb, dtype=torch.uint8, device=E.device)
    with torch.cuda.device(E.device):
        nv.call("ps_dot_topk", nv.ptr(E), nv.i64(N), nv.i32(D), nv.ptr(qidx), nv.i64(nq), nv.i32(k),
                               nv.i32(int(exclude_self)), nv.ptr(vals), nv.ptr(ids), nv.ptr(ws), nv.C.c_size_t(wsb),
                               nv.stream())
    return vals, ids


def l2_topk(X, Q, k, assign=None, probe=None):
    X = X.contiguous()
    Q = Q.to(X.device).contiguous()
    N, D = int(X.size(0)), int(X.size(1))
    nq = int(Q.size(0))
    if k < 1:
        raise ValueError(f"k must be positive, got {k}")
    dist = torch.empty((nq, k), dtype=torch.float32, device=X.device)
    ids = torch.empty((nq, k), dtype=torch.int64, device=X.device)
    L = nv.lib()
    wsb = int(L.ps_l2_topk_workspace_bytes(nv.i64(nq), nv.i64(N), nv.i32(D), nv.i32(k)))
    ws = torch.empty(wsb, dtype=torch.uint8, device=X.device)
    words = int(probe.size(1)) if probe is not None else 0
    with torch.cuda.device(X.device):
        nv.call("ps_l2_topk", nv.ptr(X), nv.i64(N), nv.i32(D), nv.ptr(Q), nv.i64(nq), nv.i32(k), nv.ptr(assign),
                nv.ptr(probe), nv.i32(words), nv.ptr(dist), nv.ptr(ids), nv.ptr(ws), nv.C.c_size_t(wsb), nv.stream())
    return dist, ids


def ivf_topk(Xs, list_ptr, item_ids, Q, probes, k, max_list=None):
    Xs = Xs.contiguous()
    Q = Q.to(Xs.device).contiguous()
    probes = probes.to(device=Xs.device, dtype=torch.int32).contiguous()
    list_ptr = list_ptr.to(device=Xs.device, dtype=torch.int64).contiguous()
    item_ids = item_ids.to(device=Xs.device, dtype=torch.int64).contiguous()
    N, D = int(Xs.size(0)), int(Xs.size(1))
    nq, nprobe, nlist = int(Q.size(0)), int(probes.size(1)), int(list_ptr.numel()) - 1
    if k < 1:
        raise ValueError(f"k must be positive, got {k}")
    if int(probes.size(0)) != nq or int(item_ids.numel()) != N or int(Q.size(1)) != D:
        raise ValueError("shape mismatch")
    if max_list is None:
        max_list = int((list_ptr[1:] - list_ptr[:-1]).max().item()) if nlist else 0
    dist = torch.empty((nq, k), dtype=torch.float32, device=Xs.device)
    ids = torch.empty((nq, k), dtype=torch.int64, device=Xs.device)
    L = nv.lib()
    wsb = int(L.ps_ivf_topk_workspace_bytes(nv.i64(nq), nv.i64(N), nv.i32(D), nv.i32(k), nv.i32(nlist), nv.i32(nprobe), nv.i64(int(max_list))))
    ws = torch.empty(wsb, dtype=torch.uint8, device=Xs.device)
    with torch.cuda.device(Xs.device):
        nv.call("ps_ivf_topk", nv.ptr(Xs), nv.i64(N), nv.i32(D), nv.ptr(list_ptr), nv.i32(nlist), nv.i64(int(max_list)), nv.ptr(item_ids),
                nv.ptr(Q), nv.i64(nq), nv.ptr(probes), nv.i32(nprobe), nv.i32(int(k)), nv.ptr(dist), nv.ptr(ids), nv.ptr(ws),
                nv.C.c_size_t(wsb), nv.stream())
    return dist, ids


_jump_polys_dev = {}


def _jump_polys(dev):
    key = str(dev)
    if key not in _jump_polys_dev:
        from . import mtjump
        import numpy as np
        _jump_polys_dev[key] = torch.from_numpy(mtjump.jump_polynomials().view(np.int32)).to(dev).contiguous()
    return _jump_polys_dev[key]


_radix_polys_dev = {}


def _radix_polys(dev):
    key = str(dev)
    if key not in _radix_polys_dev:
        from . import mtjump
        import numpy as np
        cl2 = int(nv.lib().ps_mt19937_chunk_log2())
        _radix_polys_dev[key] = torch.from_numpy(mtjump.radix_polynomials(cl2).view(np.int32)).to(dev).contiguous()
    return _radix_polys_dev[key]


_window_polys_dev = {}


def _window_polys(dev):
    key = str(dev)
    if key not in _window_polys_dev:
        from . import mtjump
        import numpy as np
        cl2 = int(nv.lib().ps_mt19937_chunk_log2())
        shift = int(nv.lib().ps_mt19937_window_shift())
        _window_polys_dev[key] = torch.from_numpy(mtjump.window_polynomials(cl2, shift=shift).view(np.int32)).to(dev).contiguous()
    return _window_polys_dev[key]


_pending_state = []


def finish_rng_state():
    import numpy as np
    while _pending_state:
        name, has_gauss, cached, host_state, host_pos, ev = _pending_state.pop()
        ev.synchronize()
        np.random.set_state((name, host_state.numpy().view(np.uint32).copy(), int(host_pos.item()), has_gauss, cached))


def mt19937_random_sample(n, device, skip=0, advance=True, parallel=True, radix=True, raw=False, one_round=True, ranges=None):
    import numpy as np
    name, key, pos, has_gauss, cached = np.random.get_state()
    if name != "MT19937":
        raise RuntimeError("numpy global RNG is not MT19937")
    dev = torch.device(device)
    if os.environ.get("PS_MT_SYNC_UPLOAD") == "1":
        st_in = torch.from_numpy(key.astype(np.uint32).view(np.int32)).to(dev)
    else:
        st_in = torch.from_numpy(key.astype(np.uint32).view(np.int32)).pin_memory().to(dev, non_blocking=True)
    st_out = torch.empty(624, dtype=torch.int32, device=dev)
    pos_out = torch.empty(1, dtype=torch.int32, device=dev)
    if raw and (skip != 0 or not parallel or n < (1 << 17)):
        raise ValueError("raw stream: skip = 0, the parallel generator and n >= 2^17 are required")
    out = (torch.empty(2 * int(n) + 1248, dtype=torch.int32, device=dev) if raw else
           torch.empty(int(n), dtype=torch.float64, device=dev))
    polys = _jump_polys(dev) if parallel else None
    rpolys = _radix_polys(dev) if (parallel and radix) else None
    wpolys = _window_polys(dev) if (parallel and radix and one_round) else None
    L = nv.lib()
    wsb = int(L.ps_mt19937_workspace_bytes(nv.i64(int(skip)), nv.i64(int(n)))) if parallel else 0
    ws = torch.empty(wsb, dtype=torch.uint8, device=dev) if parallel else None
    if ranges is not None and not raw:
        raise ValueError("ranges: raw stream only")
    rg = np.ascontiguousarray(np.asarray(ranges, dtype=np.int64).reshape(-1, 2)) if ranges is not None and len(ranges) else None
    if rg is not None and rg.shape[0] > 3:
        rg = None
    if rg is not None and os.environ.get("PS_MT_POISON") == "1":
        out.fill_(-1)
    with torch.cuda.device(dev):
        if raw:
            nv.call("ps_mt19937_raw_stream", nv.ptr(st_in), nv.i32(int(pos)), nv.i64(int(n)), nv.ptr(out), nv.ptr(st_out),
                    nv.ptr(pos_out), nv.ptr(polys), nv.i32(int(polys.size(0))), nv.ptr(rpolys),
                    nv.i32(int(rpolys.size(0)) if rpolys is not None else 0), nv.ptr(wpolys),
                    nv.i32(int(wpolys.size(0)) if wpolys is not None else 0),
                    rg.ctypes.data_as(nv.C.c_void_p) if rg is not None else nv.C.c_void_p(0), nv.i32(int(rg.shape[0]) if rg is not None else 0),
                    nv.ptr(ws), nv.C.c_size_t(wsb), nv.stream())
        else:
          nv.call("ps_mt19937_random_sample", nv.ptr(st_in), nv.i32(int(pos)), nv.i64(int(skip)), nv.i64(int(n)),
                nv.ptr(out), nv.ptr(st_out), nv.ptr(pos_out), nv.ptr(polys),
                nv.i32(int(polys.size(0)) if polys is not None else 0), nv.ptr(rpolys),
                nv.i32(int(rpolys.size(0)) if rpolys is not None else 0), nv.ptr(wpolys),
                nv.i32(int(wpolys.size(0)) if wpolys is not None else 0), nv.ptr(ws), nv.C.c_size_t(wsb), nv.stream())
    if advance == "defer":
        finish_rng_state()
        host_state = torch.empty(624, dtype=torch.int32).pin_memory()
        host_pos = torch.empty(1, dtype=torch.int32).pin_memory()
        with torch.cuda.device(dev):
            host_state.copy_(st_out, non_blocking=True)
            host_pos.copy_(pos_out, non_blocking=True)
            ev = torch.cuda.Event()
            ev.record()
        _pending_state.append((name, has_gauss, cached, host_state, host_pos, ev))
    elif advance:
        new_key = st_out.cpu().numpy().view(np.uint32)
        np.random.set_state((name, new_key, int(pos_out.item()), has_gauss, cached))
    return out
```

### movie-recommendation-engine_amd/pinsage_hip/native.py

```python
from __future__ import annotations

import ctypes as C
import os

import torch

_HERE = os.path.dirname(os.path.abspath(__file__))
SO_PATH = os.environ.get("PS_HIP_LIB") or os.path.join(_HERE, "libpinsage_hip.so")
_lib = None

PS_RNG_STREAM = 0
PS_RNG_PHILOX = 1
PS_RNG_STREAM_RAW = 2
PS_RNG_STREAM_WALKS = 3
PS_WALK_HALF_BUCKETS = 0x100
PS_RELU = 1
PS_L2NORM = 2
PS_WPERM = 4
PS_OK, PS_EINVAL, PS_ELAUNCH, PS_EWORKSPACE, PS_EUNSUPPORTED = 0, -1, -2, -3, -4


class LibraryMissing(RuntimeError):
    pass


class NativeError(RuntimeError):
    pass


SYMBOLS = [
    "ps_abi_version", "ps_error_string", "ps_csr_build_workspace_bytes", "ps_csr_build", "ps_cdf_build",
    "ps_guide_build", "ps_pack_edges", "ps_bucket_build", "ps_bucket_build_half", "ps_dest_info_build", "ps_graph_stats", "ps_walk_sample", "ps_walk_sample_layers", "ps_walk_paths", "ps_uniform_offsets", "ps_mt19937_window_shift", "ps_mt19937_workspace_bytes", "ps_mt19937_chunk_log2", "ps_mt19937_random_sample", "ps_mt19937_raw_stream",
    "ps_importance_pool", "ps_permute_k", "ps_linear", "ps_lsh_encode", "ps_hamming_topk_workspace_bytes", "ps_hamming_topk",
    "ps_lsh_planes_bytes", "ps_lsh_expand", "ps_hamming_topk_mfma_workspace_bytes", "ps_hamming_topk_mfma", "ps_hamming_topk_mfma_codes",
    "ps_topk_merge", "ps_topk_merge_strided", "ps_dot_topk_workspace_bytes", "ps_dot_topk", "ps_l2_topk_workspace_bytes", "ps_l2_topk", "ps_ivf_topk_workspace_bytes", "ps_ivf_topk", "ps_spmm_csr",
]


def have_lib() -> bool:
    return os.path.exists(SO_PATH)


def lib():
    global _lib
    if _lib is None:
        if not have_lib():
            raise LibraryMissing(
                f"{SO_PATH} not found: build it with `python -c 'import __graft_entry__ as g; g.build()'` "
                "(hipcc --offload-arch=gfx950).  There is no CPU fallback for the PinSage hot path.")
        _lib = C.CDLL(SO_PATH)
        _lib.ps_error_string.restype = C.c_char_p
        for name in ("ps_csr_build_workspace_bytes", "ps_hamming_topk_workspace_bytes", "ps_dot_topk_workspace_bytes",
                     "ps_l2_topk_workspace_bytes", "ps_ivf_topk_workspace_bytes", "ps_mt19937_workspace_bytes", "ps_lsh_planes_bytes",
                     "ps_hamming_topk_mfma_workspace_bytes"):
            if hasattr(_lib, name):
                getattr(_lib, name).restype = C.c_size_t
    return _lib


def check(rc: int, what: str):
    if rc != 0:
        raise NativeError(f"{what}: {lib().ps_error_string(rc).decode()} (code {rc})")


class KernelTimer:

    def __init__(self):
        self.events = []

    def summary(self):
        torch.cuda.synchronize()
        out = {}
        for name, a, b in self.events:
            d = out.setdefault(name, {"launches": 0, "ms": 0.0})
            d["launches"] += 1
            d["ms"] += a.elapsed_time(b)
        for d in out.values():
            d["avg_ms"] = d["ms"] / d["launches"]
        return out


_timer = None


def set_timer(t):
    global _timer
    _timer = t


def call(name, *args):
    fn = getattr(lib(), name)
    if _timer is None:
        rc = fn(*args)
    else:
        a, b = torch.cuda.Event(enable_timing=True), torch.cuda.Event(enable_timing=True)
        a.record()
        rc = fn(*args)
        b.record()
        _timer.events.append((name, a, b))
    check(rc, name)


def ptr(t):
    if t is None:
        return C.c_void_p(0)
    if not t.is_cuda:
        raise NativeError("libpinsage_hip takes device (HBM) pointers; got a CPU tensor")
    if not t.is_contiguous():
        raise NativeError("tensor must be contiguous")
    return C.c_void_p(t.data_ptr())


_raw_stream = getattr(torch._C, "_cuda_getCurrentRawStream", None)
_get_device = getattr(torch._C, "_cuda_getDevice", None)


def stream():
    if _raw_stream is not None and _get_device is not None:
        return C.c_void_p(_raw_stream(_get_device()))
    return C.c_void_p(torch.cuda.current_stream().cuda_stream)


def require_gpu():
    if not torch.cuda.is_available():
        raise NativeError("the PinSage hot path needs an MI355X (torch.cuda is not available); "
                          "there is no CPU fallback")
    lib()
    return torch.device("cuda", torch.cuda.current_device())


i64 = C.c_int64
i32 = C.c_int
u64 = C.c_uint64
u32 = C.c_uint32
```

### movie-recommendation-engine_amd/pinsage_hip/shard.py

```python
from __future__ import annotations

import os

import torch
import torch.distributed as dist

from . import dense, sampling


def shard_range(M, rank, world):
    chunk = (M + world - 1) // world
    lo = min(rank * chunk, M)
    return lo, min(lo + chunk, M), chunk


def _backend(group):
    return dist.get_backend(group) if dist.is_initialized() else None


class _Gather:

    def __init__(self, out, work=None, dev=None):
        self.out, self.work, self.dev = out, work, dev

    def wait(self):
        if self.work is not None:
            self.work.wait()
        return self.out if self.dev is None else self.out.to(self.dev)


class Comm:

    def __init__(self, group=None, standin=None):
        self.group = group
        self.standin = standin
        if standin is not None:
            self.rank, self.world = int(standin[0]), int(standin[1])
        elif dist.is_initialized():
            self.rank, self.world = dist.get_rank(group), dist.get_world_size(group)
        else:
            self.rank, self.world = 0, 1
        self._bufs = {}

    def _buf(self, kind, tag, shape, dtype, device, zero=False):
        key = (kind, tag, tuple(shape), dtype, str(device))
        b = self._bufs.get(key)
        if b is None:
            b = (torch.zeros if zero else torch.empty)(tuple(shape), dtype=dtype, device=device)
            self._bufs[key] = b
        return b

    def gather_rows_async(self, t, chunk, tag="rows"):
        if self.world == 1:
            return _Gather(t)
        rest = tuple(t.shape[1:])
        if self.standin is not None:
            key = ("recv", tag, (self.world * chunk,) + rest, t.dtype, str(t.device))
            fresh = key not in self._bufs
            out = self._buf("recv", tag, (self.world * chunk,) + rest, t.dtype, t.device, zero=True)
            for r in (range(self.world) if fresh else (self.rank,)):
                out[r * chunk: r * chunk + t.size(0)].copy_(t)
            return _Gather(out)
        if t.size(0) == chunk and t.is_contiguous():
            src = t
        else:
            src = self._buf("send", tag, (chunk,) + rest, t.dtype, t.device, zero=True)
            src[: t.size(0)].copy_(t)
        if _backend(self.group) == "gloo" and src.is_cuda:
            out = torch.empty((self.world * chunk,) + rest, dtype=t.dtype)
            dist.all_gather_into_tensor(out, src.cpu().contiguous(), group=self.group)
            return _Gather(out, dev=t.device)
        out = self._buf("recv", tag, (self.world * chunk,) + rest, t.dtype, src.device)
        work = dist.all_gather_into_tensor(out, src, group=self.group, async_op=True)
        return _Gather(out, work)

    def gather_rows(self, t, chunk, tag="rows"):
        return self.gather_rows_async(t, chunk, tag).wait()


def all_gather_rows_async(t, chunk, group=None):
    c = Comm(group)
    return c.gather_rows_async(t, chunk)


def all_gather_rows(t, chunk, group=None):
    return all_gather_rows_async(t, chunk, group).wait()


def fused_self_update(ops, P, i, H):
    Ws, bs = P[f"convs.{i}.lin_self.weight"], P[f"convs.{i}.lin_self.bias"]
    Wu, bu = P[f"convs.{i}.lin_update.weight"], P[f"convs.{i}.lin_update.bias"]
    Wu1 = Wu[:, :H].contiguous()
    W1 = ops.linear(Wu1, Ws.t().contiguous(), None)
    b1 = ops.linear(bs.reshape(1, -1).contiguous(), Wu1, bu).reshape(-1)
    return W1, b1


class HipOps:

    def sample(self, sampler, nodes, T, shard=None):
        if shard is not None and getattr(sampler, "rng", None) == "numpy":
            M, lo = shard
            all_nodes = torch.arange(M, dtype=torch.int64, device=nodes.device)
            return sampler.sample_batch(nodes, T, stream_nodes=(all_nodes, lo))
        return sampler.sample_batch(nodes, T)

    def sample_layers(self, sampler, lo, hi, T, layers, shard=None):
        stream = None
        if shard is not None and getattr(sampler, "rng", None) == "numpy":
            stream = (range(shard[0]), shard[1])
        return sampler.sample_batches(range(lo, hi), T, layers, stream_nodes=stream, defer_state=True)

    def finish(self):
        dense.finish_rng_state()

    def pool(self, h_full, batch, max_idx):
        return sampling.importance_pool(h_full, batch, max_idx=max_idx)

    def linear(self, x, W, b, x2=None, W2=None, relu=False, l2norm=False):
        return dense.linear(x, W, b, x2=x2, W2=W2, relu=relu, l2norm=l2norm)

    def lsh_encode(self, x, A):
        return dense.lsh_encode(x, A)

    def stage_weight(self, W):
        return dense.stage_weight(W)

    def lsh_planes(self, codes):
        return dense.lsh_expand(codes)

    def hamming_topk(self, q, codes, k, id_offset, planes=None, out=None):
        return dense.hamming_topk(q, codes, k, id_offset=id_offset, planes=planes, out=out)

    def topk_merge(self, d, i):
        return dense.topk_merge(d, i)

    def topk_merge_records(self, records, nq, k):
        return dense.topk_merge_records(records, nq, k)


class ShardedPinSage:

    def __init__(self, params, num_layers, sampler, num_items, ops=None, group=None, standin=None):
        self.P = params
        self.num_layers = num_layers
        self.sampler = sampler
        self.M = int(num_items)
        self.ops = ops if ops is not None else HipOps()
        self.group = group
        self.comm = Comm(group, standin=standin)
        self.rank, self.world = self.comm.rank, self.comm.world
        self.lo, self.hi, self.chunk = shard_range(self.M, self.rank, self.world)
        self._nodes = {}
        self.overlap_sampling = False
        self.overlap_input_proj = os.environ.get("PS_OVERLAP_INPUT_PROJ") == "1"
        self.fuse_self = True
        self._streams = {}
        self._fused = {}
        self._staged = {}

    def refresh_weights(self, params=None):
        if params is not None:
            self.P = params
        self._fused.clear()
        self._staged.clear()

    def _fused_layer(self, i, H):
        if i not in self._fused:
            self._fused[i] = fused_self_update(self.ops, self.P, i, H)
        return self._fused[i]

    def _w(self, key, W):
        if not hasattr(self.ops, "stage_weight"):
            return W
        t = self._staged.get(key)
        if t is None:
            t = self._staged[key] = self.ops.stage_weight(W)
        return t

    def _side_stream(self, dev):
        key = str(dev)
        if key not in self._streams:
            self._streams[key] = torch.cuda.Stream(device=dev)
        return self._streams[key]

    def _sample(self, nodes, T, shard):
        try:
            return self.ops.sample(self.sampler, nodes, T, shard)
        except TypeError:
            return self.ops.sample(self.sampler, nodes, T)

    def embed(self, x_local, T, x_full=None):
        try:
            return self._embed(x_local, T, x_full)
        finally:
            if hasattr(self.ops, "finish"):
                self.ops.finish()

    def _embed(self, x_local, T, x_full=None):
        ops, P = self.ops, self.P
        dev = x_local.device
        fused = (not (self.overlap_sampling and x_local.is_cuda)) and hasattr(ops, "sample_layers") \
            and hasattr(self.sampler, "sample_batches")
        nodes = None
        if not fused:
            nodes = self._nodes.get(str(dev))
            if nodes is None:
                nodes = self._nodes[str(dev)] = torch.arange(self.lo, self.hi, dtype=torch.int64, device=dev)
        shard = (self.M, self.lo) if self.world > 1 else None
        side = self._side_stream(dev) if (self.overlap_sampling and x_local.is_cuda) else None
        batches, ready = [], []
        early_h = None
        if (self.overlap_input_proj and fused and x_local.is_cuda and getattr(self.sampler, "rng", None) == "numpy"
                and not (x_full is not None and self.world > 1)):
            main = torch.cuda.current_stream(dev)
            aux = self._side_stream(dev)
            aux.wait_stream(main)
            with torch.cuda.stream(aux):
                early_h = ops.linear(x_local, self._w("in", P["input_proj.weight"]), P["input_proj.bias"], relu=True)
                early_ready = aux.record_event()
            early_h.record_stream(main)
        if fused:
            batches = list(ops.sample_layers(self.sampler, self.lo, self.hi, T, self.num_layers, shard))
        elif side is not None:
            main = torch.cuda.current_stream(dev)
            side.wait_stream(main)
            with torch.cuda.stream(side):
                for _ in range(self.num_layers):
                    b = self._sample(nodes, T, shard)
                    for t in (b.ids, b.counts, b.nvalid):
                        t.record_stream(main)
                    batches.append(b)
                    ready.append(side.record_event())
        else:
            batches.append(self._sample(nodes, T, shard))
        if early_h is not None:
            torch.cuda.current_stream(dev).wait_event(early_ready)
        if x_full is not None and self.world > 1:
            h_all = ops.linear(x_full, self._w("in", P["input_proj.weight"]), P["input_proj.bias"], relu=True)
            h = h_all[self.lo:self.hi]
            pending = _Gather(h_all)
        else:
            h = early_h if early_h is not None else ops.linear(x_local, self._w("in", P["input_proj.weight"]), P["input_proj.bias"], relu=True)
            pending = self.comm.gather_rows_async(h, self.chunk, "h")
        for i in range(self.num_layers):
            if side is None and not fused and i + 1 < self.num_layers:
                batches.append(self._sample(nodes, T, shard))
            H = h.size(1)
            Wu = P[f"convs.{i}.lin_update.weight"]
            if self.fuse_self:
                W1, b1 = self._fused_layer(i, H)
                a_in = h
            else:
                a_in = ops.linear(h, P[f"convs.{i}.lin_self.weight"], P[f"convs.{i}.lin_self.bias"])
                W1, b1 = Wu[:, :H], P[f"convs.{i}.lin_update.bias"]
            h_full = pending.wait()
            if side is not None:
                torch.cuda.current_stream(dev).wait_event(ready[i])
            h_neigh = ops.pool(h_full, batches[i], self.M - 1)
            h = ops.linear(a_in, self._w(("l1", i), W1), b1, x2=h_neigh, W2=self._w(("l2", i), Wu[:, H:]), relu=True, l2norm=True)
            if i + 1 < self.num_layers:
                pending = self.comm.gather_rows_async(h, self.chunk, "h")
        return ops.linear(h, self._w("out", P["output_proj.weight"]), P["output_proj.bias"], l2norm=True)

    def _staged_A(self, A):
        if not hasattr(self.ops, "stage_weight") or not isinstance(A, torch.Tensor):
            return A
        ent = self._staged.get("A")
        if ent is None or ent[0] is not A or ent[1] != A._version:
            ent = self._staged["A"] = (A, A._version, self.ops.stage_weight(A))
        return ent[2]

    REPLICATE_CODES_BYTES = 64 << 20

    def build_index(self, emb_local, A):
        self.A = A
        self.codes = self.ops.lsh_encode(emb_local, self._staged_A(A))
        self.codes_all = None
        if self.world > 1 and self.M * int(self.codes.size(1)) <= self.REPLICATE_CODES_BYTES:
            self.codes_all = self.comm.gather_rows(self.codes, self.chunk, "codes")[: self.M]
        scanned = self.codes_all if self.codes_all is not None else self.codes
        self.planes = self.ops.lsh_planes(scanned) if hasattr(self.ops, "lsh_planes") else None
        return self.codes

    def search(self, q_local, k):
        ops = self.ops
        qc = ops.lsh_encode(q_local, self._staged_A(self.A))
        nq_local = qc.size(0)
        planes = getattr(self, "planes", None)
        if self.world > 1 and getattr(self, "codes_all", None) is not None:
            n = nq_local * k
            rec = (12 * n + 15) // 16 * 16
            mine = self.comm._buf("res", "mine", (1, rec), torch.uint8, qc.device, zero=True)
            ids_v = mine[0, : 8 * n].view(torch.int64).view(nq_local, k)
            dist_v = mine[0, 8 * n: 12 * n].view(torch.int32).view(nq_local, k)
            try:
                ops.hamming_topk(qc, self.codes_all, k, 0, planes=planes, out=(dist_v, ids_v))
            except TypeError:
                d, i = ops.hamming_topk(qc, self.codes_all, k, 0)
                dist_v.copy_(d)
                ids_v.copy_(i)
            allr = self.comm.gather_rows(mine, 1, "res")
            P_ = self.world
            return (allr[:, 8 * n: 12 * n].view(torch.int32).reshape(P_ * nq_local, k),
                    allr[:, : 8 * n].view(torch.int64).reshape(P_ * nq_local, k))
        qc_all = self.comm.gather_rows(qc, nq_local, "qcodes")
        if self.world == 1:
            return (ops.hamming_topk(qc_all, self.codes, k, self.lo, planes=planes) if planes is not None
                    else ops.hamming_topk(qc_all, self.codes, k, self.lo))
        nq = qc_all.size(0)
        n = nq * k
        rec = (12 * n + 15) // 16 * 16
        mine = self.comm._buf("cand", "mine", (1, rec), torch.uint8, qc_all.device, zero=True)
        ids_v = mine[0, : 8 * n].view(torch.int64).view(nq, k)
        dist_v = mine[0, 8 * n: 12 * n].view(torch.int32).view(nq, k)
        try:
            ops.hamming_topk(qc_all, self.codes, k, self.lo, planes=planes, out=(dist_v, ids_v))
        except TypeError:
            d, i = ops.hamming_topk(qc_all, self.codes, k, self.lo)
            dist_v.copy_(d)
            ids_v.copy_(i)
        allc = self.comm.gather_rows(mine, 1, "cand")
        if hasattr(ops, "topk_merge_records"):
            return ops.topk_merge_records(allc, nq, k)
        d_all = torch.stack([allc[p, 8 * n: 12 * n].view(torch.int32).view(nq, k) for p in range(self.world)])
        i_all = torch.stack([allc[p, : 8 * n].view(torch.int64).view(nq, k) for p in range(self.world)])
        return ops.topk_merge(d_all, i_all)
```

Before: 42.90 million items/s.

## Fuse importance pooling into GCN layer GEMM with heavy-row reordering

Adds a ps_gcn_layer entry point that computes neighbour importance pooling inside the layer GEMM kernel. Count and order kernels first partition rows into those with kept neighbours and those without. Tiles of rows with neighbours pool into a per-block workspace slab that feeds the second GEMM operand, while the other tiles skip that operand entirely. Output rows are scattered back through the permutation. This removes the separate pooled h_neigh tensor and its extra kernel launch, at the cost of two small prepass kernels, indirect row loads, permuted stores, and a workspace the size of M×H.

```diff
diff --git a/include/pinsage_hip.h b/include/pinsage_hip.h
--- a/include/pinsage_hip.h
+++ b/include/pinsage_hip.h
@@ -96,6 +96,12 @@
 int ps_linear(const float *x, int64_t M, int K, const float *W, int ldw, const float *b, int N,
               const float *x2, int K2, const float *W2, int ldw2, int flags, float *y, ps_stream_t stream);
 
+size_t ps_gcn_layer_workspace_bytes(int64_t M, int H);
+int ps_gcn_layer(const float *x, int64_t M, int K, const float *W, int ldw, const float *b, int N, const float *h_full,
+                 int64_t n_full, int H, const int32_t *ids, const int32_t *counts, const float *wts, const int32_t *nvalid,
+                 int T, int64_t max_idx, int renorm, const float *W2, int ldw2, int flags, float *y, void *workspace,
+                 size_t workspace_bytes, ps_stream_t stream);
+
 int ps_lsh_encode(const float *x, int64_t N, int D, const float *A, int nbits, uint8_t *codes, int flags, ps_stream_t stream);
 
 size_t ps_hamming_topk_workspace_bytes(int64_t nq, int64_t N, int cs, int k);
diff --git a/movie-recommendation-engine_amd/csrc/dense_mfma.hip b/movie-recommendation-engine_amd/csrc/dense_mfma.hip
--- a/movie-recommendation-engine_amd/csrc/dense_mfma.hip
+++ b/movie-recommendation-engine_amd/csrc/dense_mfma.hip
@@ -1,4 +1,5 @@
 #include "ps_common.h"
+#include "pool_row.h"
 #include <type_traits>
 
 #ifndef PS_GEMM_DEBUG
@@ -34,6 +35,9 @@
     float *y;
     uint8_t *codes; int cs;
     const int64_t *grp;
+    const int32_t *ord; const int32_t *nheavy; float *slab;
+    const float *hf; int H; const int32_t *ids; const int32_t *counts; const float *wts; const int32_t *nvalid; int T; int renorm;
+    int64_t max_idx;
 };
 
 __device__ __forceinline__ void load8(const float *base, bool row_ok, int k, int K, bool vec_ok, float (&v)[8]) {
@@ -106,8 +110,9 @@
     *reinterpret_cast<f32x4 *>(d + 4) = hi;
 }
 
-template <int WM, int WN, int TM, int TN, int EPI>
-__device__ __forceinline__ void gemm_epilogue(const GemmArgs &g, f32x16 (&acc)[TM][TN], int64_t m0, int n0, float *sRed, float *sNrm) {
+template <int WM, int WN, int TM, int TN, int EPI, bool PERM = false>
+__device__ __forceinline__ void gemm_epilogue(const GemmArgs &g, f32x16 (&acc)[TM][TN], int64_t m0, int n0, float *sRed, float *sNrm,
+                                              const int *sOrd = nullptr) {
     constexpr int BM = WM * TM * 32, BN = WN * TN * 32, NT = WM * WN * 64;
     const int tid = threadIdx.x, lane = tid & 63, wv = tid >> 6;
     const int wm = wv / WN, wn = wv % WN, li = lane & 31, lh = lane >> 5;
@@ -238,6 +243,7 @@
 #pragma unroll
             for (int r = 0; r < 16; ++r) {
                 float *dst = g.y + (m0 + (wm * TM + a) * 32 + (r & 3) + 8 * (r >> 2) + 4 * lh) * g.N + n0 + wn * TN * 32 + li;
+                if constexpr (PERM) dst = g.y + (int64_t)sOrd[(wm * TM + a) * 32 + (r & 3) + 8 * (r >> 2) + 4 * lh] * g.N + n0 + wn * TN * 32 + li;
 #pragma unroll
                 for (int b = 0; b < TN; ++b) dst[b * 32] = acc[a][b][r];
             }
@@ -248,8 +254,9 @@
     for (int a = 0; a < TM; ++a)
 #pragma unroll
         for (int r = 0; r < 16; ++r) {
-            const int64_t row = m0 + (wm * TM + a) * 32 + (r & 3) + 8 * (r >> 2) + 4 * lh;
+            int64_t row = m0 + (wm * TM + a) * 32 + (r & 3) + 8 * (r >> 2) + 4 * lh;
             if (row >= g.M) continue;
+            if constexpr (PERM) row = sOrd[(wm * TM + a) * 32 + (r & 3) + 8 * (r >> 2) + 4 * lh];
 #pragma unroll
             for (int b = 0; b < TN; ++b) {
                 const int col = n0 + (wn * TN + b) * 32 + li;
@@ -259,7 +266,7 @@
     PS_TRACE(41);
 }
 
-template <int WM, int WN, int TM, int TN, int BK, int EPI, bool FAST>
+template <int WM, int WN, int TM, int TN, int BK, int EPI, bool FAST, int GCN = 0>
 #ifndef PS_GEMM_OCC
 #define PS_GEMM_OCC 2
 #endif
@@ -270,8 +277,9 @@
     constexpr int GRP = BK / 8;
     constexpr int LDS_STRIDE = BK + 4;
     constexpr int A_ITEMS = (BM * GRP + NT - 1) / NT, B_ITEMS = (BN * GRP + NT - 1) / NT;
-    __shared__ __attribute__((aligned(16))) float smem[(BM + BN) * LDS_STRIDE + BM * WN + BM * 4];
+    __shared__ __attribute__((aligned(16))) float smem[(BM + BN) * LDS_STRIDE + BM * WN + BM * 4 + (GCN ? BM : 0)];
     float *sA = smem, *sB = smem + BM * LDS_STRIDE, *sRed = smem + (BM + BN) * LDS_STRIDE, *sNrm = sRed + BM * WN;
+    int *sOrd = reinterpret_cast<int *>(sNrm + BM * 4);
 
     const int tid = threadIdx.x, lane = tid & 63, wv = tid >> 6;
     const int wm = wv / WN, wn = wv % WN;
@@ -295,6 +303,29 @@
     int trace_step = 0;
 #endif
     PS_TRACE(0);
+    int64_t xrow[A_ITEMS];
+    (void)xrow;
+    if constexpr (GCN > 0) {
+        static_assert(FAST && EPI == 0 && BM == 64 && NT == 256, "the 64-row tile of the layer GEMM");
+        const bool heavy = m0 < (int64_t)*g.nheavy;
+        if (tid < BM) sOrd[tid] = g.ord[m0 + tid < g.M ? m0 + tid : g.M - 1];
+        if (heavy) {
+            float *slab = g.slab + (int64_t)blockIdx.x * BM * g.H;
+#pragma unroll 1
+            for (int r0 = 0; r0 < BM; r0 += NT / 16) {
+                const int r = r0 + (tid >> 4);
+                const bool rok = m0 + r < g.M;
+                const int64_t i = rok ? (int64_t)g.ord[m0 + r] : 0;
+                pool4_row<GCN>(g.hf, g.H, g.ids, g.counts, g.wts, g.nvalid, i, rok, g.T, g.max_idx, g.renorm, slab + (int64_t)r * g.H);
+            }
+            g.x2 = slab;
+        } else {
+            g.x2 = nullptr;
+        }
+        __syncthreads();
+#pragma unroll
+        for (int q = 0; q < A_ITEMS; ++q) xrow[q] = sOrd[((tid + NT * q) % (BM * GRP)) / GRP];
+    }
     f32x16 acc[TM][TN];
 #pragma unroll
     for (int a = 0; a < TM; ++a)
@@ -320,7 +351,9 @@
                 const int it = FAST ? (tid + NT * q) % (BM * GRP) : tid + NT * q, row = it / GRP, grp = it % GRP;
                 const int64_t m = m0 + row;
                 if (FAST) {
-                    const float *src = X + (m < g.M ? m : g.M - 1) * K + k0 + grp * 8;
+                    int64_t srow = m < g.M ? m : g.M - 1;
+                    if constexpr (GCN > 0) srow = phase == 0 ? xrow[q] : srow - m0;
+                    const float *src = X + srow * K + k0 + grp * 8;
                     ra[q][0] = *reinterpret_cast<const f32x4 *>(src);
                     ra[q][1] = *reinterpret_cast<const f32x4 *>(src + 4);
                 } else if (it < BM * GRP) {
@@ -413,7 +446,7 @@
         }
     }
 
-    gemm_epilogue<WM, WN, TM, TN, EPI>(g, acc, m0, n0, sRed, sNrm);
+    gemm_epilogue<WM, WN, TM, TN, EPI, (GCN > 0)>(g, acc, m0, n0, sRed, sNrm, sOrd);
 }
 
 template <int WM, int WN, int TM, int TN, int BK, int EPI>
@@ -1054,6 +1087,133 @@
     return PS_OK;
 }
 
+namespace {
+
+constexpr int GCN_MAX_CHUNKS = 1024;
+
+int64_t gcn_chunk_rows(int64_t M) {
+    const int64_t c = ps_cdiv(ps_cdiv(M, GCN_MAX_CHUNKS), 256) * 256;
+    return c > 256 ? c : 256;
+}
+
+struct GcnWorkspace {
+    size_t slab, ord, cnt, total;
+};
+GcnWorkspace gcn_workspace(int64_t M, int H) {
+    GcnWorkspace w;
+    w.slab = 0;
+    w.ord = (size_t)ps_cdiv(M, 64) * 64 * (size_t)H * sizeof(float);
+    w.cnt = w.ord + (size_t)ps_cdiv(M, 64) * 64 * sizeof(int32_t);
+    w.total = w.cnt + (GCN_MAX_CHUNKS + 64) * sizeof(int32_t);
+    return w;
+}
+
+__global__ __launch_bounds__(256) void gcn_count_kernel(const int32_t *__restrict__ ids, const int32_t *__restrict__ nvalid, int64_t M,
+                                                        int T, int64_t max_idx, int64_t chunk, int32_t *__restrict__ cnt) {
+    __shared__ int sw[4];
+    const int tid = threadIdx.x, lane = tid & 63, wv = tid >> 6;
+    const int64_t r0 = (int64_t)blockIdx.x * chunk, r1 = r0 + chunk < M ? r0 + chunk : M;
+    int c = 0;
+    for (int64_t i = r0 + tid; i < r1; i += 256) c += pool_row_keeps(ids, nvalid, i, T, max_idx) ? 1 : 0;
+    c = ps_wave_sum_i32(c);
+    if (lane == 0) sw[wv] = c;
+    __syncthreads();
+    if (tid == 0) cnt[blockIdx.x] = sw[0] + sw[1] + sw[2] + sw[3];
+}
+
+__global__ __launch_bounds__(256) void gcn_order_kernel(const int32_t *__restrict__ ids, const int32_t *__restrict__ nvalid, int64_t M,
+                                                        int T, int64_t max_idx, int64_t chunk, int nchunks,
+                                                        const int32_t *__restrict__ cnt, int32_t *__restrict__ ord,
+                                                        int32_t *__restrict__ nheavy) {
+    __shared__ int sb[4], st[4], sh[4], se[4];
+    const int tid = threadIdx.x, lane = tid & 63, wv = tid >> 6;
+    const int64_t r0 = (int64_t)blockIdx.x * chunk, r1 = r0 + chunk < M ? r0 + chunk : M;
+    int before = 0, total = 0;
+    for (int j = tid; j < nchunks; j += 256) {
+        const int v = cnt[j];
+        total += v;
+        before += j < (int)blockIdx.x ? v : 0;
+    }
+    before = ps_wave_sum_i32(before);
+    total = ps_wave_sum_i32(total);
+    if (lane == 0) { sb[wv] = before; st[wv] = total; }
+    __syncthreads();
+    before = sb[0] + sb[1] + sb[2] + sb[3];
+    total = st[0] + st[1] + st[2] + st[3];
+    if (blockIdx.x == 0 && tid == 0) *nheavy = total;
+    int64_t hoff = before, eoff = total + (r0 - before);
+    for (int64_t base = r0; base < r1; base += 256) {
+        const int64_t i = base + tid;
+        const bool in = i < r1;
+        const bool f = in && pool_row_keeps(ids, nvalid, i, T, max_idx);
+        const uint64_t hm = __ballot(f), em = __ballot(in && !f);
+        const int hr = (int)__builtin_amdgcn_mbcnt_hi((uint32_t)(hm >> 32), __builtin_amdgcn_mbcnt_lo((uint32_t)hm, 0u));
+        const int er = (int)__builtin_amdgcn_mbcnt_hi((uint32_t)(em >> 32), __builtin_amdgcn_mbcnt_lo((uint32_t)em, 0u));
+        if (lane == 0) { sh[wv] = __popcll(hm); se[wv] = __popcll(em); }
+        __syncthreads();
+        int hb = 0, eb = 0, ht = 0, et = 0;
+#pragma unroll
+        for (int w = 0; w < 4; ++w) {
+            hb += w < wv ? sh[w] : 0;
+            eb += w < wv ? se[w] : 0;
+            ht += sh[w];
+            et += se[w];
+        }
+        if (in) ord[f ? hoff + hb + hr : eoff + eb + er] = (int32_t)i;
+        hoff += ht;
+        eoff += et;
+        __syncthreads();
+    }
+}
+
+bool env_set(const char *name) {
+    const char *e = getenv(name);
+    return e != nullptr && *e != '\0';
+}
+
+}
+
+extern "C" size_t ps_gcn_layer_workspace_bytes(int64_t M, int H) {
+    if (M <= 0 || H <= 0) return 0;
+    return gcn_workspace(M, H).total;
+}
+
+extern "C" int ps_gcn_layer(const float *x, int64_t M, int K, const float *W, int ldw, const float *b, int N, const float *h_full,
+                            int64_t n_full, int H, const int32_t *ids, const int32_t *counts, const float *wts, const int32_t *nvalid,
+                            int T, int64_t max_idx, int renorm, const float *W2, int ldw2, int flags, float *y, void *workspace,
+                            size_t workspace_bytes, ps_stream_t stream) {
+    if (M < 0 || K <= 0 || N <= 0 || ldw < K || H <= 0 || ldw2 < H || T <= 0 || n_full < 0) return PS_EINVAL;
+    if (flags & ~(PS_RELU | PS_L2NORM | PS_WPERM)) return PS_EINVAL;
+    if (M > 0 && (!x || !W || !y || !h_full || !W2 || !ids || !nvalid || (!counts && !wts))) return PS_EINVAL;
+    const char *fe = getenv("PS_GCN_FUSED");
+    const char *se = getenv("PS_GEMM_SHARD"), *pe = getenv("PS_POOL_ROWS_PER_WAVE");
+    if ((fe && atoi(fe) == 0) || (se && atoi(se) > 0) || env_set("PS_GEMM_DMA") || (pe && atoi(pe) == 1)) return PS_EUNSUPPORTED;
+    if (N != 256 || (flags & (PS_RELU | PS_L2NORM)) != (PS_RELU | PS_L2NORM) || M < 64 * 384 || M > 0x7fffffff - 64 || T > 16)
+        return PS_EUNSUPPORTED;
+    if (!aligned_operand(x, K, K) || !aligned_operand(W, K, ldw) || !aligned_operand(W2, H, ldw2) || !aligned_operand(h_full, H, H))
+        return PS_EUNSUPPORTED;
+    const GcnWorkspace wl = gcn_workspace(M, H);
+    if (!workspace || workspace_bytes < wl.total || reinterpret_cast<size_t>(workspace) % 16 != 0) return PS_EWORKSPACE;
+    if (max_idx > n_full - 1) max_idx = n_full - 1;
+    unsigned char *ws = static_cast<unsigned char *>(workspace);
+    int32_t *ord = reinterpret_cast<int32_t *>(ws + wl.ord), *cnt = reinterpret_cast<int32_t *>(ws + wl.cnt);
+    int32_t *nheavy = cnt + GCN_MAX_CHUNKS;
+    hipStream_t st = ps_stream(stream);
+    const int64_t chunk = gcn_chunk_rows(M);
+    const int nchunks = (int)ps_cdiv(M, chunk);
+    hipLaunchKernelGGL(gcn_count_kernel, dim3((unsigned)nchunks), dim3(256), 0, st, ids, nvalid, M, T, max_idx, chunk, cnt);
+    PS_CHECK_LAUNCH();
+    hipLaunchKernelGGL(gcn_order_kernel, dim3((unsigned)nchunks), dim3(256), 0, st, ids, nvalid, M, T, max_idx, chunk, nchunks, cnt, ord,
+                       nheavy);
+    PS_CHECK_LAUNCH();
+    GemmArgs g{x, M, K, W, ldw, nullptr, H, W2, ldw2, b, N, flags, y, nullptr, 0, nullptr,
+               ord, nheavy, reinterpret_cast<float *>(ws + wl.slab), h_full, H, ids, counts, wts, nvalid, T, renorm, max_idx};
+    const dim3 grid((unsigned)ps_cdiv(M, 64), 1);
+    hipLaunchKernelGGL((gemm_f32_kernel<1, 4, 2, 2, 32, 0, true, 1>), grid, dim3(256), 0, st, g);
+    PS_CHECK_LAUNCH();
+    return PS_OK;
+}
+
 __global__ void permute_k_kernel(const float *__restrict__ W, int64_t rows, int K, int ld, float *__restrict__ out) {
     const int64_t total = rows * (K / 8);
     for (int64_t i = (int64_t)blockIdx.x * blockDim.x + threadIdx.x; i < total; i += (int64_t)gridDim.x * blockDim.x) {
diff --git a/movie-recommendation-engine_amd/csrc/importance_pool.hip b/movie-recommendation-engine_amd/csrc/importance_pool.hip
--- a/movie-recommendation-engine_amd/csrc/importance_pool.hip
+++ b/movie-recommendation-engine_amd/csrc/importance_pool.hip
@@ -1,4 +1,5 @@
 #include "ps_common.h"
+#include "pool_row.h"
 
 namespace {
 
@@ -108,109 +109,17 @@
     }
 }
 
-template <int CTRL>
-__device__ __forceinline__ int row_bcast_i32(int v) { return __builtin_amdgcn_update_dpp(0, v, CTRL, 0xf, 0xf, false); }
-__device__ __forceinline__ int row16_sum_i32(int v) {
-    v += __builtin_amdgcn_update_dpp(0, v, 0xB1, 0xf, 0xf, true);
-    v += __builtin_amdgcn_update_dpp(0, v, 0x4E, 0xf, 0xf, true);
-    v += __builtin_amdgcn_update_dpp(0, v, 0x141, 0xf, 0xf, true);
-    v += __builtin_amdgcn_update_dpp(0, v, 0x140, 0xf, 0xf, true);
-    return v;
-}
-__device__ __forceinline__ float row16_sum_f32(float v) {
-    v += __builtin_bit_cast(float, __builtin_amdgcn_update_dpp(0, __builtin_bit_cast(int, v), 0xB1, 0xf, 0xf, true));
-    v += __builtin_bit_cast(float, __builtin_amdgcn_update_dpp(0, __builtin_bit_cast(int, v), 0x4E, 0xf, 0xf, true));
-    v += __builtin_bit_cast(float, __builtin_amdgcn_update_dpp(0, __builtin_bit_cast(int, v), 0x141, 0xf, 0xf, true));
-    v += __builtin_bit_cast(float, __builtin_amdgcn_update_dpp(0, __builtin_bit_cast(int, v), 0x140, 0xf, 0xf, true));
-    return v;
-}
-
 template <int PAGES>
 __global__ __launch_bounds__(256) void importance_pool4_kernel(const float *__restrict__ x, int H, const int32_t *__restrict__ ids,
                                                                const int32_t *__restrict__ counts, const float *__restrict__ wts,
                                                                const int32_t *__restrict__ nvalid, int64_t B, int T, int64_t max_idx,
                                                                int renorm, float *__restrict__ out) {
-    constexpr int TU = 4;
-    const int lane = threadIdx.x & 63, l = lane & 15, g = lane >> 4;
+    const int lane = threadIdx.x & 63, g = lane >> 4;
     const int64_t wave0 = ((int64_t)blockIdx.x * blockDim.x + threadIdx.x) >> 6;
     const int64_t nwaves = ((int64_t)gridDim.x * blockDim.x) >> 6;
     for (int64_t i0 = wave0 * 4; i0 < B; i0 += nwaves * 4) {
         const int64_t i = i0 + g;
-        const bool rok = i < B;
-        int k = rok ? nvalid[i] : 0;
-        int32_t id[PAGES], cn[PAGES];
-        float w[PAGES];
-#pragma unroll
-        for (int p = 0; p < PAGES; ++p) {
-            const int e = p * 16 + l;
-            const bool in = rok && e < T;
-            id[p] = in ? ids[i * T + e] : -1;
-            cn[p] = (in && counts) ? counts[i * T + e] : 0;
-            w[p] = (in && wts) ? wts[i * T + e] : 0.f;
-        }
-        k = k < T ? k : T;
-        int tot = 0;
-#pragma unroll
-        for (int p = 0; p < PAGES; ++p) tot += (p * 16 + l < k) ? cn[p] : 0;
-        tot = row16_sum_i32(tot);
-        float wsum = 0.f;
-#pragma unroll
-        for (int p = 0; p < PAGES; ++p) {
-            const bool keep = (p * 16 + l < k) && id[p] >= 0 && (int64_t)id[p] <= max_idx;
-            w[p] = keep ? (wts ? w[p] : (float)((double)cn[p] / (double)tot)) : 0.f;
-            id[p] = keep ? id[p] : -1;
-            wsum += w[p];
-        }
-        wsum = row16_sum_f32(wsum);
-        if (renorm && wsum > 0.f) {
-#pragma unroll
-            for (int p = 0; p < PAGES; ++p) w[p] = id[p] >= 0 ? w[p] / wsum : 0.f;
-        }
-        int kmax = __builtin_amdgcn_readlane(k, 0);
-        { const int k1 = __builtin_amdgcn_readlane(k, 16), k2 = __builtin_amdgcn_readlane(k, 32), k3 = __builtin_amdgcn_readlane(k, 48);
-          kmax = kmax > k1 ? kmax : k1; kmax = kmax > k2 ? kmax : k2; kmax = kmax > k3 ? kmax : k3; }
-        for (int cb = 0; cb < H; cb += 256) {
-            float4 acc[4];
-#pragma unroll
-            for (int s = 0; s < 4; ++s) acc[s] = make_float4(0.f, 0.f, 0.f, 0.f);
-#define PS_POOL_ENTRY(P, TT, U)                                                                            \
-            {                                                                                              \
-                nid[U] = row_bcast_i32<0x150 + (TT)>(id[P]);                                               \
-                nw[U] = __builtin_bit_cast(float, row_bcast_i32<0x150 + (TT)>(__builtin_bit_cast(int, w[P]))); \
-                _Pragma("unroll") for (int s = 0; s < 4; ++s) {                                            \
-                    const int col = cb + s * 64 + l * 4;                                                   \
-                    r[U][s] = make_float4(0.f, 0.f, 0.f, 0.f);                                             \
-                    if (nid[U] >= 0 && col < H) r[U][s] = *reinterpret_cast<const float4 *>(x + (int64_t)nid[U] * H + col); \
-                }                                                                                          \
-            }
-#define PS_POOL_BATCH(P, T0)                                                                               \
-            if ((P) * 16 + (T0) < kmax) {                                                                  \
-                int32_t nid[TU];                                                                           \
-                float nw[TU];                                                                              \
-                float4 r[TU][4];                                                                           \
-                PS_POOL_ENTRY(P, (T0) + 0, 0) PS_POOL_ENTRY(P, (T0) + 1, 1) PS_POOL_ENTRY(P, (T0) + 2, 2) PS_POOL_ENTRY(P, (T0) + 3, 3) \
-                _Pragma("unroll") for (int u = 0; u < TU; ++u)                                             \
-                    _Pragma("unroll") for (int s = 0; s < 4; ++s) {                                        \
-                        acc[s].x = fmaf(r[u][s].x, nw[u], acc[s].x); acc[s].y = fmaf(r[u][s].y, nw[u], acc[s].y); \
-                        acc[s].z = fmaf(r[u][s].z, nw[u], acc[s].z); acc[s].w = fmaf(r[u][s].w, nw[u], acc[s].w); \
-                    }                                                                                      \
-            }
-#define PS_POOL_PAGE(P) PS_POOL_BATCH(P, 0) PS_POOL_BATCH(P, 4) PS_POOL_BATCH(P, 8) PS_POOL_BATCH(P, 12)
-            PS_POOL_PAGE(0)
-            if constexpr (PAGES > 1) { PS_POOL_PAGE(1) }
-            if constexpr (PAGES > 2) { PS_POOL_PAGE(2) }
-            if constexpr (PAGES > 3) { PS_POOL_PAGE(3) }
-#undef PS_POOL_PAGE
-#undef PS_POOL_BATCH
-#undef PS_POOL_ENTRY
-            if (rok) {
-#pragma unroll
-                for (int s = 0; s < 4; ++s) {
-                    const int col = cb + s * 64 + l * 4;
-                    if (col < H) *reinterpret_cast<float4 *>(out + i * H + col) = acc[s];
-                }
-            }
-        }
+        pool4_row<PAGES>(x, H, ids, counts, wts, nvalid, i, i < B, T, max_idx, renorm, out + i * H);
     }
 }
 
diff --git a/movie-recommendation-engine_amd/csrc/pool_row.h b/movie-recommendation-engine_amd/csrc/pool_row.h
--- /dev/null
+++ b/movie-recommendation-engine_amd/csrc/pool_row.h
@@ -0,0 +1,122 @@
+#pragma once
+#include "ps_common.h"
+
+namespace {
+
+template <int CTRL>
+__device__ __forceinline__ int row_bcast_i32(int v) { return __builtin_amdgcn_update_dpp(0, v, CTRL, 0xf, 0xf, false); }
+__device__ __forceinline__ int row16_sum_i32(int v) {
+    v += __builtin_amdgcn_update_dpp(0, v, 0xB1, 0xf, 0xf, true);
+    v += __builtin_amdgcn_update_dpp(0, v, 0x4E, 0xf, 0xf, true);
+    v += __builtin_amdgcn_update_dpp(0, v, 0x141, 0xf, 0xf, true);
+    v += __builtin_amdgcn_update_dpp(0, v, 0x140, 0xf, 0xf, true);
+    return v;
+}
+__device__ __forceinline__ float row16_sum_f32(float v) {
+    v += __builtin_bit_cast(float, __builtin_amdgcn_update_dpp(0, __builtin_bit_cast(int, v), 0xB1, 0xf, 0xf, true));
+    v += __builtin_bit_cast(float, __builtin_amdgcn_update_dpp(0, __builtin_bit_cast(int, v), 0x4E, 0xf, 0xf, true));
+    v += __builtin_bit_cast(float, __builtin_amdgcn_update_dpp(0, __builtin_bit_cast(int, v), 0x141, 0xf, 0xf, true));
+    v += __builtin_bit_cast(float, __builtin_amdgcn_update_dpp(0, __builtin_bit_cast(int, v), 0x140, 0xf, 0xf, true));
+    return v;
+}
+
+__device__ __forceinline__ bool pool_row_keeps(const int32_t *__restrict__ ids, const int32_t *__restrict__ nvalid, int64_t i, int T,
+                                               int64_t max_idx) {
+    int k = nvalid[i];
+    k = k < T ? k : T;
+    bool keep = false;
+    for (int j0 = 0; j0 < T; j0 += 16) {
+        int32_t v[16];
+#pragma unroll
+        for (int u = 0; u < 16; ++u) v[u] = j0 + u < T ? ids[i * T + j0 + u] : -1;
+#pragma unroll
+        for (int u = 0; u < 16; ++u) keep |= j0 + u < k && v[u] >= 0 && (int64_t)v[u] <= max_idx;
+        if (keep || j0 + 16 >= k) break;
+    }
+    return keep;
+}
+
+template <int PAGES>
+__device__ __forceinline__ void pool4_row(const float *__restrict__ x, int H, const int32_t *__restrict__ ids,
+                                          const int32_t *__restrict__ counts, const float *__restrict__ wts,
+                                          const int32_t *__restrict__ nvalid, int64_t i, bool rok, int T, int64_t max_idx, int renorm,
+                                          float *__restrict__ orow) {
+    constexpr int TU = 4;
+    const int lane = threadIdx.x & 63, l = lane & 15;
+    int k = rok ? nvalid[i] : 0;
+    int32_t id[PAGES], cn[PAGES];
+    float w[PAGES];
+#pragma unroll
+    for (int p = 0; p < PAGES; ++p) {
+        const int e = p * 16 + l;
+        const bool in = rok && e < T;
+        id[p] = in ? ids[i * T + e] : -1;
+        cn[p] = (in && counts) ? counts[i * T + e] : 0;
+        w[p] = (in && wts) ? wts[i * T + e] : 0.f;
+    }
+    k = k < T ? k : T;
+    int tot = 0;
+#pragma unroll
+    for (int p = 0; p < PAGES; ++p) tot += (p * 16 + l < k) ? cn[p] : 0;
+    tot = row16_sum_i32(tot);
+    float wsum = 0.f;
+#pragma unroll
+    for (int p = 0; p < PAGES; ++p) {
+        const bool keep = (p * 16 + l < k) && id[p] >= 0 && (int64_t)id[p] <= max_idx;
+        w[p] = keep ? (wts ? w[p] : (float)((double)cn[p] / (double)tot)) : 0.f;
+        id[p] = keep ? id[p] : -1;
+        wsum += w[p];
+    }
+    wsum = row16_sum_f32(wsum);
+    if (renorm && wsum > 0.f) {
+#pragma unroll
+        for (int p = 0; p < PAGES; ++p) w[p] = id[p] >= 0 ? w[p] / wsum : 0.f;
+    }
+    int kmax = __builtin_amdgcn_readlane(k, 0);
+    { const int k1 = __builtin_amdgcn_readlane(k, 16), k2 = __builtin_amdgcn_readlane(k, 32), k3 = __builtin_amdgcn_readlane(k, 48);
+      kmax = kmax > k1 ? kmax : k1; kmax = kmax > k2 ? kmax : k2; kmax = kmax > k3 ? kmax : k3; }
+    for (int cb = 0; cb < H; cb += 256) {
+        float4 acc[4];
+#pragma unroll
+        for (int s = 0; s < 4; ++s) acc[s] = make_float4(0.f, 0.f, 0.f, 0.f);
+#define PS_POOL_ENTRY(P, TT, U)                                                                            \
+        {                                                                                                  \
+            nid[U] = row_bcast_i32<0x150 + (TT)>(id[P]);                                                   \
+            nw[U] = __builtin_bit_cast(float, row_bcast_i32<0x150 + (TT)>(__builtin_bit_cast(int, w[P]))); \
+            _Pragma("unroll") for (int s = 0; s < 4; ++s) {                                                \
+                const int col = cb + s * 64 + l * 4;                                                       \
+                r[U][s] = make_float4(0.f, 0.f, 0.f, 0.f);                                                 \
+                if (nid[U] >= 0 && col < H) r[U][s] = *reinterpret_cast<const float4 *>(x + (int64_t)nid[U] * H + col); \
+            }                                                                                              \
+        }
+#define PS_POOL_BATCH(P, T0)                                                                               \
+        if ((P) * 16 + (T0) < kmax) {                                                                      \
+            int32_t nid[TU];                                                                               \
+            float nw[TU];                                                                                  \
+            float4 r[TU][4];                                                                               \
+            PS_POOL_ENTRY(P, (T0) + 0, 0) PS_POOL_ENTRY(P, (T0) + 1, 1) PS_POOL_ENTRY(P, (T0) + 2, 2) PS_POOL_ENTRY(P, (T0) + 3, 3) \
+            _Pragma("unroll") for (int u = 0; u < TU; ++u)                                                 \
+                _Pragma("unroll") for (int s = 0; s < 4; ++s) {                                            \
+                    acc[s].x = fmaf(r[u][s].x, nw[u], acc[s].x); acc[s].y = fmaf(r[u][s].y, nw[u], acc[s].y); \
+                    acc[s].z = fmaf(r[u][s].z, nw[u], acc[s].z); acc[s].w = fmaf(r[u][s].w, nw[u], acc[s].w); \
+                }                                                                                          \
+        }
+#define PS_POOL_PAGE(P) PS_POOL_BATCH(P, 0) PS_POOL_BATCH(P, 4) PS_POOL_BATCH(P, 8) PS_POOL_BATCH(P, 12)
+        PS_POOL_PAGE(0)
+        if constexpr (PAGES > 1) { PS_POOL_PAGE(1) }
+        if constexpr (PAGES > 2) { PS_POOL_PAGE(2) }
+        if constexpr (PAGES > 3) { PS_POOL_PAGE(3) }
+#undef PS_POOL_PAGE
+#undef PS_POOL_BATCH
+#undef PS_POOL_ENTRY
+        if (rok) {
+#pragma unroll
+            for (int s = 0; s < 4; ++s) {
+                const int col = cb + s * 64 + l * 4;
+                if (col < H) *reinterpret_cast<float4 *>(orow + col) = acc[s];
+            }
+        }
+    }
+}
+
+}
diff --git a/movie-recommendation-engine_amd/pinsage_hip/dense.py b/movie-recommendation-engine_amd/pinsage_hip/dense.py
--- a/movie-recommendation-engine_amd/pinsage_hip/dense.py
+++ b/movie-recommendation-engine_amd/pinsage_hip/dense.py
@@ -86,6 +86,49 @@
                                     nv.ptr(x2), nv.i32(K2), _ptr_view(W2k), nv.i32(ldw2), nv.i32(flags), nv.ptr(y),
                                     nv.stream())
     return y
+
+
+def gcn_layer(x, W, b, h_full, ids, counts, nvalid, W2, wts=None, max_idx=None, renorm=True, relu=True, l2norm=True):
+    from . import sampling
+    staged = isinstance(W, StagedWeight)
+    if isinstance(W2, StagedWeight) != staged:
+        raise ValueError("W and W2 must both be staged or both plain")
+    Wm, W2m = (W.t, W2.t) if staged else (W, W2)
+    _require_cuda(x, Wm, b, h_full, W2m, ids, counts, wts, nvalid)
+    x, h_full = x.contiguous(), h_full.contiguous()
+    if x.dtype != torch.float32 or h_full.dtype != torch.float32:
+        raise TypeError("fp32 expected")
+    M, K = int(x.size(0)), int(x.size(1))
+    n_full, H = int(h_full.size(0)), int(h_full.size(1))
+    Wk, ldw = _rowmajor(Wm)
+    W2k, ldw2 = _rowmajor(W2m)
+    N = int(Wk.size(0))
+    if int(Wk.size(1)) != K or int(W2k.size(1)) != H or int(W2k.size(0)) != N or int(ids.size(0)) != M:
+        raise ValueError("shape mismatch")
+    T = int(ids.size(1))
+    if max_idx is None:
+        max_idx = n_full - 1
+    if b is not None:
+        b = b.contiguous()
+    ids, nvalid = ids.contiguous(), nvalid.contiguous()
+    counts = counts.contiguous() if counts is not None else None
+    wts = wts.contiguous() if wts is not None else None
+    flags = (nv.PS_RELU if relu else 0) | (nv.PS_L2NORM if l2norm else 0) | (nv.PS_WPERM if staged else 0)
+    L = nv.lib()
+    wsb = int(L.ps_gcn_layer_workspace_bytes(nv.i64(M), nv.i32(H)))
+    if wsb > 0:
+        y = torch.empty((M, N), dtype=torch.float32, device=x.device)
+        ws = torch.empty((wsb,), dtype=torch.uint8, device=x.device)
+        with torch.cuda.device(x.device):
+            rc = L.ps_gcn_layer(nv.ptr(x), nv.i64(M), nv.i32(K), _ptr_view(Wk), nv.i32(ldw), nv.ptr(b), nv.i32(N), nv.ptr(h_full),
+                                nv.i64(n_full), nv.i32(H), nv.ptr(ids), nv.ptr(counts), nv.ptr(wts), nv.ptr(nvalid), nv.i32(T),
+                                nv.i64(int(max_idx)), nv.i32(int(renorm)), _ptr_view(W2k), nv.i32(ldw2), nv.i32(flags), nv.ptr(y),
+                                nv.ptr(ws), nv.C.c_size_t(wsb), nv.stream())
+        if rc != nv.PS_EUNSUPPORTED:
+            nv.check(rc, "ps_gcn_layer")
+            return y
+    h_neigh = sampling.importance_pool(h_full, ids=ids, counts=counts, wts=wts, nvalid=nvalid, max_idx=max_idx, renorm=renorm)
+    return linear(x, W, b, x2=h_neigh, W2=W2, relu=relu, l2norm=l2norm)
 
 
 def lsh_encode(x, A):
diff --git a/movie-recommendation-engine_amd/pinsage_hip/native.py b/movie-recommendation-engine_amd/pinsage_hip/native.py
--- a/movie-recommendation-engine_amd/pinsage_hip/native.py
+++ b/movie-recommendation-engine_amd/pinsage_hip/native.py
@@ -31,7 +31,7 @@
 SYMBOLS = [
     "ps_abi_version", "ps_error_string", "ps_csr_build_workspace_bytes", "ps_csr_build", "ps_cdf_build",
     "ps_guide_build", "ps_pack_edges", "ps_bucket_build", "ps_bucket_build_half", "ps_dest_info_build", "ps_graph_stats", "ps_walk_sample", "ps_walk_sample_layers", "ps_walk_paths", "ps_uniform_offsets", "ps_mt19937_window_shift", "ps_mt19937_workspace_bytes", "ps_mt19937_chunk_log2", "ps_mt19937_random_sample", "ps_mt19937_raw_stream",
-    "ps_importance_pool", "ps_permute_k", "ps_linear", "ps_lsh_encode", "ps_hamming_topk_workspace_bytes", "ps_hamming_topk",
+    "ps_importance_pool", "ps_permute_k", "ps_linear", "ps_gcn_layer_workspace_bytes", "ps_gcn_layer", "ps_lsh_encode", "ps_hamming_topk_workspace_bytes", "ps_hamming_topk",
     "ps_lsh_planes_bytes", "ps_lsh_expand", "ps_hamming_topk_mfma_workspace_bytes", "ps_hamming_topk_mfma", "ps_hamming_topk_mfma_codes",
     "ps_topk_merge", "ps_topk_merge_strided", "ps_dot_topk_workspace_bytes", "ps_dot_topk", "ps_l2_topk_workspace_bytes", "ps_l2_topk", "ps_ivf_topk_workspace_bytes", "ps_ivf_topk", "ps_spmm_csr",
 ]
@@ -52,7 +52,7 @@
         _lib.ps_error_string.restype = C.c_char_p
         for name in ("ps_csr_build_workspace_bytes", "ps_hamming_topk_workspace_bytes", "ps_dot_topk_workspace_bytes",
                      "ps_l2_topk_workspace_bytes", "ps_ivf_topk_workspace_bytes", "ps_mt19937_workspace_bytes", "ps_lsh_planes_bytes",
-                     "ps_hamming_topk_mfma_workspace_bytes"):
+                     "ps_hamming_topk_mfma_workspace_bytes", "ps_gcn_layer_workspace_bytes"):
             if hasattr(_lib, name):
                 getattr(_lib, name).restype = C.c_size_t
     return _lib
diff --git a/movie-recommendation-engine_amd/pinsage_hip/shard.py b/movie-recommendation-engine_amd/pinsage_hip/shard.py
--- a/movie-recommendation-engine_amd/pinsage_hip/shard.py
+++ b/movie-recommendation-engine_amd/pinsage_hip/shard.py
@@ -119,6 +119,9 @@
 
     def linear(self, x, W, b, x2=None, W2=None, relu=False, l2norm=False):
         return dense.linear(x, W, b, x2=x2, W2=W2, relu=relu, l2norm=l2norm)
+
+    def gcn_layer(self, x, W, b, h_full, batch, max_idx, W2):
+        return dense.gcn_layer(x, W, b, h_full, batch.ids, batch.counts, batch.nvalid, W2, max_idx=max_idx)
 
     def lsh_encode(self, x, A):
         return dense.lsh_encode(x, A)
@@ -257,8 +260,11 @@
             h_full = pending.wait()
             if side is not None:
                 torch.cuda.current_stream(dev).wait_event(ready[i])
-            h_neigh = ops.pool(h_full, batches[i], self.M - 1)
-            h = ops.linear(a_in, self._w(("l1", i), W1), b1, x2=h_neigh, W2=self._w(("l2", i), Wu[:, H:]), relu=True, l2norm=True)
+            if self.fuse_self and hasattr(ops, "gcn_layer"):
+                h = ops.gcn_layer(a_in, self._w(("l1", i), W1), b1, h_full, batches[i], self.M - 1, self._w(("l2", i), Wu[:, H:]))
+            else:
+                h_neigh = ops.pool(h_full, batches[i], self.M - 1)
+                h = ops.linear(a_in, self._w(("l1", i), W1), b1, x2=h_neigh, W2=self._w(("l2", i), Wu[:, H:]), relu=True, l2norm=True)
             if i + 1 < self.num_layers:
                 pending = self.comm.gather_rows_async(h, self.chunk, "h")
         return ops.linear(h, self._w("out", P["output_proj.weight"]), P["output_proj.bias"], l2norm=True)
```

Measured after the change: 45.03 million items/s, median of 6. 5.0% higher.
